# jxhe/vae-lagging-encoder

Measured on AMD Instinct MI355X. Metric: aggressive-loop seqs/sec, higher is better.
Workload: dtype bf16

## Files before the change

include/lvae.h:

```cpp
#ifndef LVAE_H
#define LVAE_H

#include <stdint.h>

#ifdef __cplusplus
extern "C" {
#endif

int lv_gemm_f32(int transA, int transB, int M, int N, int K, float alpha,
                const float* A, long lda, const float* B, long ldb, float* C, long ldc, int accumulate,
                const float* add1, long ld1, int mod1, const float* add2, long ld2, int mod2,
                float* ws , long ws_floats, void* stream);

int lv_gemm_bf16(int transA, int transB, int M, int N, int K, float alpha,
                 const float* A, long lda, const float* B, long ldb, float* C, long ldc, int accumulate,
                 const float* add1, long ld1, int mod1, const float* add2, long ld2, int mod2,
                 float* ws, long ws_floats, void* stream);

int lv_gemm_b16(int transA, int M, int N, int K, float alpha,
                const uint16_t* A, long lda, const uint16_t* B, long ldb, float* C, long ldc, int accumulate,
                const float* add1, long ld1, int mod1, const float* add2, long ld2, int mod2,
                float* ws, long ws_floats, void* stream);
int lv_gemm_b16_dual_supported(int M, int N, int K, long ws_floats);
int lv_gemm_b16_dual(int transA, int M, int N, int K, const uint16_t* A, long lda, const uint16_t* B, long ldb,
// ... 208 lines not shown

int lv_tanh_f32(const float* in, float* out, long n, void* stream);
int lv_colsum_f32(const float* in, long ld, int R, int C, float* out, float* out2, void* stream);
int lv_add_f32(const float* a, const float* b, float* out, long n, void* stream);
int lv_sum_accum_f32(const float* x, long n, float* out_dev, void* stream);
int lv_add_scalar_f32(float* x_dev, float v, void* stream);

int lv_sumsq_workspace_floats(void);
int lv_sumsq_f32(const float* x, long n, float* ws, float* out_dev, int accumulate, void* stream);
int lv_clip_coef_f32(const float* sumsq_dev, float max_norm, float* coef_dev, float* norm_out_dev, void* stream);
int lv_clip_norm2_f32(const float* g1, long n1, const float* g2, long n2, float* ws, float max_norm,
                      float* sumsq_dev, float* coef_dev, float* norm_dev, void* stream);
int lv_sgd_step_f32(float* p, float* g, long n, const float* lr_dev, const float* coef_dev, int write_back_clipped,
                    void* stream);
int lv_scale_f32(float* x, long n, const float* coef_dev, void* stream);
int lv_clip_norm2_txn_f32(const float* g1, long n1, const float* g2, long n2, float* ws, float max_norm,
                          float* sumsq_dev, float* coef_dev, float* norm_dev, const int* status1, const int* status2,
                          const float* guard, float* txn, float* acc, void* stream);
int lv_clip_norm2_fold_txn_f32(const float* g1, long n1, const float* g2, long n2, float* ws, const float* extra, int n_extra,
                               float max_norm, float* sumsq_dev, float* coef_dev, float* norm_dev, const int* status1,
                               const int* status2, const float* guard, float* txn, float* acc, void* stream);
int lv_clip_coef_txn_f32(const float* sumsq_dev, float max_norm, float* coef_dev, float* norm_out_dev, const int* status1,
                         const int* status2, const float* guard, float* txn, float* acc, void* stream);
int lv_txn_guard_f32(const int* status1, const int* status2, float* guard, void* stream);
int lv_sgd_step_txn_f32(float* p, float* g, long n, const float* lr_dev, const float* coef_dev, int write_back_clipped,
                        const float* void_flag_dev, void* stream);
int lv_scale_txn_f32(float* x, long n, const float* coef_dev, const float* void_flag_dev, void* stream);
int lv_sgd_step_scale_txn_f32(float* p, float* g, long n, const float* lr_dev, const float* coef_dev, int write_back_clipped,
                              float* x2, long n2, const float* void_flag_dev, void* stream);
int lv_sgd_step_scale_rows_txn_f32(float* p, float* g, long n, const float* lr_dev, const float* coef_dev, int write_back_clipped,
                                   float* x2, long n2, const float* void_flag_dev, long emb_off, int V, int ni, const int* sorted_tok,
                                   int N, void* stream);
int lv_sgd_momentum_step_f32(float* p, float* g, float* buf, long n, const float* lr_dev, const float* coef_dev, float momentum,
                             int write_back_clipped, void* stream);
int lv_sgd_momentum_step_txn_f32(float* p, float* g, float* buf, long n, const float* lr_dev, const float* coef_dev, float momentum,
                                 int write_back_clipped, const float* void_flag_dev, void* stream);
int lv_sgd_momentum_step_scale_txn_f32(float* p, float* g, float* buf, long n, const float* lr_dev, const float* coef_dev, float momentum,
                                       int write_back_clipped, float* x2, long n2, const float* void_flag_dev, void* stream);
int lv_adam_step_f32(float* p, float* g, float* m, float* v, long n, const float* lr_dev, const float* coef_dev,
                     const float* step_dev, float beta1, float beta2, float eps, int write_back_clipped, void* stream);
int lv_adam_step_txn_f32(float* p, float* g, float* m, float* v, long n, const float* lr_dev, const float* coef_dev, float* step_dev,
                         double beta1, double beta2, float eps, int write_back_clipped, const float* void_flag_dev, void* stream);
int lv_adam_step_scale_txn_f32(float* p, float* g, float* m, float* v, long n, const float* lr_dev, const float* coef_dev,
                               float* step_dev, double beta1, double beta2, float eps, int write_back_clipped, float* x2, long n2,
                               const float* void_flag_dev, void* stream);

int lv_rng_normal_f32(float* out, long n, const uint64_t* state_dev, uint64_t substream, void* stream);
int lv_rng_keepmask_u8(uint8_t* out, long n, float keep_prob, const uint64_t* state_dev, uint64_t substream, void* stream);
int lv_rng_advance(uint64_t* state_dev, uint64_t inc, void* stream);
int lv_rng_noise_step(float* eps, long n_eps, uint8_t* mask_in, long n_in, float keep_in, uint8_t* mask_out, long n_out,
                      float keep_out, uint64_t* state_dev, uint64_t inc, void* stream);
int lv_rng_bernoulli_f32(const float* p, float* out, long n, const uint64_t* state_dev, uint64_t substream,
                         void* stream);

int lv_gauss_logpdf_f32(const float* z, const float* mu, const float* logvar, float* out, int B, int ns, int nz, void* stream);
int lv_logsumexp_rows_f32(const float* in, long ld, int R, int C, float add, float* out, void* stream);
int lv_calc_mi_f32(const float* mu, const float* logvar, const float* z, float* ws, float* out_dev, int Bx, int Bz, int nz,
                   void* stream);
int lv_au_accum_f32(const float* mu, const float* mean, float* acc_dev, int B, int nz, void* stream);

int lv_dec_cond_ll_f32_supported(int V, int ni, int H, int nz, int T);
long lv_dec_cond_ll_f32_ws_floats(int V, int H, int nz, int B, int T);
int lv_dec_cond_ll_f32(const int64_t* x, int B, int T, const float* z, long z_stride, int K, const float* embed,
                       const float* trans, const float* w_ih, const float* w_hh, const float* b_ih, const float* b_hh,
                       const float* pred, int V, int ni, int H, int nz, float* ws, float* cond_ll, void* stream);
int lv_grid_posterior_f32(const float* cond_ll, const float* z, long z_stride, int B, int K, int nz, float* log_post,
                          float* mean, void* stream);

int lv_mh_chain_f32_supported(int V, int ni, int H, int nz, int T);
long lv_mh_chain_f32_ws_floats(int V, int H, int nz, int B, int T);
int lv_mh_chain_prep_f32(const int64_t* x, int B, int T, const float* embed, const float* trans, const float* w_ih,
                         const float* w_hh, const float* b_ih, const float* b_hh, const float* pred, int V, int ni, int H, int nz,
                         float* ws, void* stream);
int lv_mh_chain_f32(const int64_t* x, int B, int T, const float* ws, int V, int H, int nz, int C, float* cur, float* cur_ll,
                    int* accepts, const float* eps, const float* u, int n_iter, int iter0, int burn_in, int thin, int nsamples,
                    float std, int first, float* samples, float* ratio_out, int* accept_out, void* stream);
int lv_mh_step_f32(const float* cond_ll, float* prop, float* cur, float* cur_ll, int* accepts, const float* u,
                   const float* eps_next, float std, float* samples, int rows, int C, int nz, int nsamples, int keep, int init,
                   float* ratio_out, int* accept_out, void* stream);

int lv_ais_chain_f32_supported(int V, int ni, int H, int nz, int T);
int lv_ais_chain_f32(const int64_t* x, int B, int T, const float* ws, int V, int H, int nz, int C, float* cur, float* g_cur,
                     float* lq_cur, double* logw, int* accepts, const float* eps, const float* u, const double* beta,
                     const float* std_it, const float* mu0, const float* lv0, int n_iter, int first, float* ratio_out,
                     int* accept_out, double* logw_out, void* stream);
int lv_ais_step_f32(const float* cond_ll, float* prop, float* cur, float* g_cur, float* lq_cur, double* logw, int* accepts,
                    const float* u, double beta, const float* eps_next, float std_next, double dbeta_next, const float* mu0,
                    const float* lv0, int rows, int C, int nz, int init, float* ratio_out, int* accept_out,
                    double* logw_out_next, void* stream);

int lv_hmc_leap_f32(const float* rec, const float* dz, int parts, float* pos, float* mom, float* k0, float* cur, float* g_cur,
                    float* lq_cur, float* rec_cur, float* d_cur, double* logw, int* accepts, float* eps, const float* u,
                    const float* mom_next, double beta, double beta_next, double dbeta_next, const float* mu0, const float* lv0,
                    int rows, int C, int nz, int L, int mode, float up, float down, float eps_min, float eps_max, float* dh_out,
                    int* flag_out, double* logw_out_next, float* keep_out, void* stream);

int lv_argmax_rows_f32(const float* in, long ld, int R, int C, int64_t* idx, void* stream);
int lv_log_softmax_rows_f32(const float* in, long ld, int R, int C, const float* addrow, float* out, long ldo, void* stream);
int lv_sample_rows_f32(const float* in, long ld, int R, int C, const float* u, int64_t* idx, void* stream);
int lv_sample_filtered_rows_f32(const float* in, long ld, int R, int C, const float* u, float inv_temp, int top_k, float top_p,
                                int64_t* idx, float* lp, float* lq, int* kept, float* tau, int* ntie, void* stream);

int lv_im2col_f32(const float* x, float* col, long ldcol, int N, int H, int W, int C, int Ho, int Wo,
                  int kh, int kw, int pad, int stride, int ntaps, void* stream);
int lv_col2im_f32(const float* dcol, long ldcol, float* dx, int N, int H, int W, int C, int Ho, int Wo,
                  int kh, int kw, int pad, int stride, int ntaps, int accumulate, void* stream);
// ... 104 lines not shown
```

vae_lagging_encoder_amd/_lib.py:

```python
import ctypes
import os
import threading

from . import build as _build

_vp = ctypes.c_void_p
_i = ctypes.c_int
_l = ctypes.c_long
_f = ctypes.c_float
_d = ctypes.c_double
_u64 = ctypes.c_uint64

SIGNATURES = {
    "lv_gemm_f32": [_i, _i, _i, _i, _i, _f, _vp, _l, _vp, _l, _vp, _l, _i, _vp, _l, _i, _vp, _l, _i, _vp, _l, _vp],
    "lv_gemm_bf16": [_i, _i, _i, _i, _i, _f, _vp, _l, _vp, _l, _vp, _l, _i, _vp, _l, _i, _vp, _l, _i, _vp, _l, _vp],
    "lv_gemm_b16": [_i, _i, _i, _i, _f, _vp, _l, _vp, _l, _vp, _l, _i, _vp, _l, _i, _vp, _l, _i, _vp, _l, _vp],
    "lv_gemm_h16": [_i, _i, _i, _f, _vp, _l, _vp, _l, _vp, _l, _i, _vp, _l, _i, _vp, _l, _i, _vp, _l, _vp],
    "lv_gemm_b16_dual_supported": [_i, _i, _i, _l],
    "lv_gemm_b16_dual": [_i, _i, _i, _i, _vp, _l, _vp, _l, _vp, _l, _i, _vp, _l, _vp, _l, _vp],
    "lv_gemm_b16_pair_supported": [_i, _i, _i, _i, _i, _i, _i, _i, _l],
    "lv_gemm_b16_pair_pending": [_vp, _vp],
    "lv_gemm_b16_pair": [_i, _i, _i, _i, _vp, _l, _vp, _l, _vp, _l, _i, _vp, _l,
                         _i, _i, _i, _i, _vp, _l, _vp, _l, _vp, _l, _vp, _l, _vp],
    "lv_gemm_b16_keep": [_i, _i, _i, _vp, _l, _vp, _l, _vp, _vp, _f, _i, _vp, _l, _vp],
    "lv_gemm_b16_sumsq_parts": [_i, _i, _i, _l],
    "lv_gemm_b16_sumsq": [_i, _i, _i, _i, _vp, _l, _vp, _l, _vp, _l, _vp, _l, _vp, _i, _vp],
    "lv_gemm_b16_nll_parts": [_i],
    "lv_gemm_b16_tile": [_i, _i, _i, _i, _i, _f, _vp, _l, _vp, _l, _vp, _l, _i, _vp, _l, _i, _vp, _l, _i, _vp, _l, _vp],
    "lv_gemm_b16_nll_tile": [_i, _i, _i, _i, _vp, _l, _vp, _l, _vp, _l, _vp, _l, _i, _i, _vp, _vp, _vp],
    "lv_gemm_b16_nll": [_i, _i, _i, _vp, _l, _vp, _l, _vp, _l, _vp, _l, _i, _i, _vp, _vp, _vp],
    "lv_softmax_nll_merge_f32": [_vp, _i, _vp, _vp, _vp, _i, _vp],
    "lv_softmax_nll_bwd_h16": [_vp, _l, _vp, _vp, _l, _i, _vp, _vp, _l, _i, _i, _i, _vp],
    "lv_cvt_bf16_f32": [_vp, _l, _i, _i, _vp, _l, _vp, _l, _vp],
    "lv_cvt_bf16_keep_f32": [_vp, _l, _i, _i, _i, _vp, _f, _vp, _l, _vp, _l, _vp],
    "lv_cvt_bf16_hs3_f32": [_vp, _l, _i, _i, _i, _vp, _f, _vp, _l, _vp, _l, _vp, _l, _vp],
    "lv_cvt_f32_bf16_scaled": [_vp, _l, _f, _vp, _vp],
    "lv_keep_scale_f32": [_vp, _vp, _f, _i, _i, _i, _vp],
    "lv_cvt_bf16_gates_f32": [_vp, _l, _i, _i, _vp, _l, _vp, _l, _vp],
    "lv_cvt_bf16_lo_f32": [_vp, _l, _i, _i, _i, _vp, _l, _i, _i, _vp, _l, _vp, _l, _vp],
    "lv_cvt_h16_f32": [_vp, _l, _i, _i, _i, _vp, _l, _i, _i, _vp, _l, _vp, _l, _vp],
    "lv_gate_interleave_f32": [_vp, _vp, _i, _i, _vp, _vp],
    "lv_lstm_fwd_bf16_ug": [_vp, _vp, _vp, _vp, _vp, _vp, _f, _vp, _vp, _i, _i, _i, _vp],
    "lv_lstm_fwd_f32_ug": [_vp, _vp, _vp, _vp, _vp, _vp, _f, _vp, _vp, _i, _i, _i, _vp],
    "lv_loss_assemble_f32": [_vp, _vp, _vp, _vp, _vp, _vp, _vp, _vp, _vp, _i, _i, _vp],
    "lv_loss_assemble_rng_f32": [_vp, _vp, _vp, _vp, _vp, _vp, _vp, _vp, _vp, _i, _i, _vp, _u64, _vp],
    "lv_gx_expand_add_f32": [_vp, _vp, _vp, _i, _i, _i, _i, _vp],
    "lv_sample_sum_f32": [_vp, _vp, _i, _i, _i, _i, _vp],
    "lv_sample_sum_b16": [_vp, _l, _vp, _l, _i, _i, _i, _i, _vp],
    "lv_repeat_rows_i64": [_vp, _vp, _i, _i, _i, _vp],
    "lv_loss_assemble_ns_f32": [_vp, _vp, _vp, _vp, _vp, _vp, _vp, _vp, _vp, _i, _i, _i, _vp],
    "lv_loss_assemble_ns_rng_f32": [_vp, _vp, _vp, _vp, _vp, _vp, _vp, _vp, _vp, _i, _i, _i, _vp, _u64, _vp],
    "lv_loss_assemble_iw_f32": [_vp] * 13 + [_i, _i, _i, _i, _vp],
    "lv_loss_assemble_iw_rng_f32": [_vp] * 13 + [_i, _i, _i, _i, _vp, _u64, _vp],
    "lv_reparam_iw_bwd_f32": [_vp, _vp, _vp, _vp, _i, _i, _i, _vp],
    "lv_enc_head_iw_bwd_f32": [_vp, _vp, _vp, _i, _vp, _vp, _vp, _vp, _vp, _vp, _i, _i, _i, _i, _vp],
    "lv_loss_assemble_dreg_f32": [_vp] * 14 + [_i, _i, _i, _i, _vp],
    "lv_loss_assemble_dreg_rng_f32": [_vp] * 14 + [_i, _i, _i, _i, _vp, _u64, _vp],
    "lv_reparam_iwdz_bwd_f32": [_vp, _vp, _vp, _vp, _vp, _vp, _i, _i, _i, _vp],
    "lv_enc_head_dreg_bwd_f32": [_vp, _vp, _vp, _i, _vp, _vp, _vp, _vp, _vp, _vp, _vp, _i, _i, _i, _i, _vp],
    "lv_kl_freebits_fwd_f32": [_vp, _f, _i, _vp, _vp, _vp, _i, _i, _vp],
    "lv_reparam_kl_gated_bwd_f32": [_vp, _vp, _vp, _vp, _vp, _vp, _i, _i, _i, _vp],
    "lv_loss_assemble_fb_f32": [_vp] * 10 + [_i, _i, _i, _vp],
    "lv_loss_assemble_fb_rng_f32": [_vp] * 10 + [_i, _i, _i, _vp, _u64, _vp],
    "lv_enc_head_gated_bwd_f32": [_vp, _vp, _vp, _i, _vp, _vp, _vp, _vp, _vp, _vp, _vp, _i, _i, _i, _i, _vp],
    "lv_enc_head_fwd_f32": [_vp, _vp, _vp, _vp, _vp, _vp, _i, _i, _i, _i, _vp],
    "lv_enc_head_bwd_f32": [_vp, _vp, _vp, _i, _vp, _vp, _vp, _vp, _vp, _vp, _i, _i, _i, _i, _vp],
    "lv_dec_tail_parts": [_i],
    "lv_dec_init_f32": [_vp, _vp, _vp, _l, _i, _vp, _vp, _vp, _vp, _vp, _i, _i, _i, _i, _vp],
    "lv_dec_tail_bwd_f32": [_vp, _vp, _vp, _vp, _l, _i, _vp, _vp, _l, _vp, _vp, _vp, _vp, _i, _i, _i, _vp],
    "lv_dec_tail_dz_f32": [_vp, _vp, _vp, _l, _i, _vp, _vp, _i, _i, _i, _vp],
    "lv_svi_step_f32": [_vp, _vp, _i, _vp, _vp, _vp, _f, _f, _f, _vp, _vp, _vp, _vp, _vp, _vp, _vp, _i, _i, _i, _vp],
    "lv_svi_rec_step_f32": [_vp, _i, _vp, _vp, _f, _f, _f, _vp, _vp, _vp, _vp, _vp, _vp, _i, _i, _i, _vp],
    "lv_savae_adjoint_f32": [_vp, _vp, _vp, _vp, _vp, _f, _f, _f, _f, _vp, _vp, _vp, _vp, _i, _i, _i, _vp],
    "lv_savae_hvp_f32": [_vp, _i, _vp, _vp, _vp, _vp, _vp, _vp, _i, _i, _i, _vp],
    "lv_clip_norm2_f32": [_vp, _l, _vp, _l, _vp, _f, _vp, _vp, _vp, _vp],
    "lv_clip_norm2_txn_f32": [_vp, _l, _vp, _l, _vp, _f, _vp, _vp, _vp, _vp, _vp, _vp, _vp, _vp, _vp],
    "lv_clip_norm2_fold_txn_f32": [_vp, _l, _vp, _l, _vp, _vp, _i, _f, _vp, _vp, _vp, _vp, _vp, _vp, _vp, _vp, _vp],
    "lv_clip_coef_txn_f32": [_vp, _f, _vp, _vp, _vp, _vp, _vp, _vp, _vp, _vp],
    "lv_txn_guard_f32": [_vp, _vp, _vp, _vp],
    "lv_sgd_step_txn_f32": [_vp, _vp, _l, _vp, _vp, _i, _vp, _vp],
    "lv_scale_txn_f32": [_vp, _l, _vp, _vp, _vp],
    "lv_sgd_step_scale_txn_f32": [_vp, _vp, _l, _vp, _vp, _i, _vp, _l, _vp, _vp],
    "lv_sgd_step_scale_rows_txn_f32": [_vp, _vp, _l, _vp, _vp, _i, _vp, _l, _vp, _l, _i, _i, _vp, _i, _vp],
    "lv_sgd_momentum_step_f32": [_vp, _vp, _vp, _l, _vp, _vp, _f, _i, _vp],
    "lv_sgd_momentum_step_txn_f32": [_vp, _vp, _vp, _l, _vp, _vp, _f, _i, _vp, _vp],
    "lv_sgd_momentum_step_scale_txn_f32": [_vp, _vp, _vp, _l, _vp, _vp, _f, _i, _vp, _l, _vp, _vp],
    "lv_rng_noise_step": [_vp, _l, _vp, _l, _f, _vp, _l, _f, _vp, _u64, _vp],
    "lv_lstm_persist16_wpk_floats": [],
    "lv_lstm_persist16_xch_floats": [],
    "lv_lstm_persist16_xch_clear": [_vp, _vp],
    "lv_lstm_persist16_saved_floats": [_i, _i],
    "lv_lstm_persist16_pack": [_vp, _vp, _i, _i, _vp],
    "lv_lstm_persist16_import_saved": [_vp, _vp, _vp, _i, _i, _i, _i, _vp],
    "lv_lstm_persist16_pack2": [_vp, _vp, _vp, _i, _vp],
# ... 213 lines not shown
```

vae_lagging_encoder_amd/csrc/lv_gemm_b16.hip:

```cpp
#if defined(LV_TRACE)
#define lv_trace_buf lv_trace_buf_gemm
#endif
#include "lv_device.h"
#if defined(LV_TRACE) && !defined(LV_EMU)
__device__ unsigned long long* lv_trace_buf = nullptr;
extern "C" int lv_trace_set_gemm(void* p) { return (int)hipMemcpyToSymbol(HIP_SYMBOL(lv_trace_buf), &p, sizeof(p)); }
#endif
#include <type_traits>

namespace {

#ifndef LV_B16_ABL
#define LV_B16_ABL 0
#endif
#ifndef LV_B16_SPLIT_TARGET
#define LV_B16_SPLIT_TARGET 512
#endif

constexpr int BK = 64;
constexpr int BT = 128;
constexpr int NCH = BK / 8;

#ifndef LV_NLL_ABL
#define LV_NLL_ABL 0
#endif
struct GemmQ {
    const uint16_t* A; const uint16_t* B; float* C;
    int M, N, K;
    long lda, ldb, ldc;
    float alpha;
    int accumulate;
    const float* add1; long ld1; int mod1;
    const float* add2; long ld2; int mod2;
    int tilesM, tilesN;
    int splits, kt_per_split;
    float* ws;
    uint16_t* C16; long ldc16;
    const int64_t* ids; long ids_stride; int tgt_off; int Bsz;
    float2* part; int nparts;
    float* tgt;
    const uint8_t* keep; float kscale; int keepT;
    float* sq; int sq_only;
    float* C2; long ldc2; int nsplit;
};

__device__ __forceinline__ uint4 load_chunk(const uint16_t* __restrict__ p, int valid) {
    if (valid >= 8) return *reinterpret_cast<const uint4*>(p);
    uint32_t h[8];
#pragma unroll
    for (int e = 0; e < 8; ++e) h[e] = e < valid ? (uint32_t)p[e] : 0u;
    uint4 q;
    q.x = h[0] | (h[1] << 16); q.y = h[2] | (h[3] << 16); q.z = h[4] | (h[5] << 16); q.w = h[6] | (h[7] << 16);
    return q;
}


// ... 1505 lines not shown
            }
            sr[u] = grs[u] < R ? grs[u] : R - 1;
        }
        if (gids) {
#pragma unroll
            for (int u = 0; u < 8; ++u) sr[u] = gids[(long)bbs[u] * gstride + (grs[u] < R ? tts[u] : 0)];
#pragma unroll
            for (int u = 0; u < 8; ++u) sr[u] = sr[u] < 0 ? 0 : (sr[u] >= gV ? gV - 1 : sr[u]);
        }
        float v[8];
        uint8_t kp[8];
#pragma unroll
        for (int u = 0; u < 8; ++u) v[u] = src[sr[u] * lds_ + gcc];
        if (keep) {
#pragma unroll
            for (int u = 0; u < 8; ++u) kp[u] = keep[((long)bbs[u] * Tt + (grs[u] < R ? tts[u] : 0)) * C + gcc];
        }
#pragma unroll
        for (int u = 0; u < 8; ++u) {
            const int gr = grs[u];
            uint16_t b = 0;
            if (gr < R && gc < C) {
                float x = v[u];
                if (keep) {
                    if (gids) x = kp[u] ? x * kscale : 0.f;
                    else x *= kp[u] ? kscale : 0.f;
                }
                b = (uint16_t)lv_f32_to_bf16_bits(x);
                if (lo == 1) b = (uint16_t)lv_f32_to_bf16_bits(x - lv_bf16_bits_to_f32(b));
                if (dst) {
                    const long dr = gate_H > 0 ? (long)(gr % gate_H) * 4 + gr / gate_H : gr;
                    dst[dr * ldd + gc] = lo == 2 ? lv_f32_to_f16_bits(lv_sat_f16(x)) : b;
                }
            }
            tile[q + 4 * (i0 + u)][lane] = b;
        }
    }
    if (!dstT) return;
    __syncthreads();
#pragma unroll 4
    for (int i = 0; i < 16; ++i) {
        const int c = q + 4 * i;
        const int gc = c0 + c, gr = r0 + lane;
        if (gc < C && gr < R) dstT[(long)gc * ldt + gr] = tile[lane][c];
    }
}


__global__ __launch_bounds__(256) void cvt_b16_v4_kernel(const float* __restrict__ src, long lds_, int R, int C,
                                                         uint16_t* __restrict__ dst, long ldd, uint16_t* __restrict__ dstT, long ldt,
                                                         int gate_H, const uint8_t* __restrict__ keep, float kscale, int Bsz,
                                                         const int64_t* __restrict__ gids, long gstride, int gV, int lo) {
    __shared__ __attribute__((aligned(8))) uint16_t tile[64][68];
    const int t = (int)threadIdx.x;
    const int r0 = (int)blockIdx.y * 64, c0 = (int)blockIdx.x * 64;
    const int q = t >> 4, cl = t & 15;
    const bool tb = keep || gids;
    const int Tt = tb ? R / Bsz : 1;
    int bb = tb ? (r0 + q) % Bsz : 0, tt = tb ? (r0 + q) / Bsz : 0;
    const int gc = c0 + 4 * cl;
    const int gcc = gc < C ? gc : C - 4;
    int grs[4], bbs[4], tts[4];
    long sr[4];
#pragma unroll
    for (int u = 0; u < 4; ++u) {
        grs[u] = r0 + q + 16 * u;
        bbs[u] = bb; tts[u] = tt;
        if (tb) {
            bb += 16;
            while (bb >= Bsz) { bb -= Bsz; ++tt; }
        }
        sr[u] = grs[u] < R ? grs[u] : R - 1;
    }
    if (gids) {
#pragma unroll
        for (int u = 0; u < 4; ++u) sr[u] = gids[(long)bbs[u] * gstride + (grs[u] < R ? tts[u] : 0)];
#pragma unroll
        for (int u = 0; u < 4; ++u) sr[u] = sr[u] < 0 ? 0 : (sr[u] >= gV ? gV - 1 : sr[u]);
    }
    float4 v[4];
    uint32_t kp[4] = {0u, 0u, 0u, 0u};
#pragma unroll
    for (int u = 0; u < 4; ++u) v[u] = *reinterpret_cast<const float4*>(src + sr[u] * lds_ + gcc);
    if (keep) {
#pragma unroll
        for (int u = 0; u < 4; ++u)
            kp[u] = *reinterpret_cast<const uint32_t*>(keep + ((long)bbs[u] * Tt + (grs[u] < R ? tts[u] : 0)) * C + gcc);
    }
#pragma unroll
    for (int u = 0; u < 4; ++u) {
        const int gr = grs[u];
        uint16_t b[4] = {0, 0, 0, 0}, d[4] = {0, 0, 0, 0};
        const bool in = gr < R && gc < C;
        if (in) {
            const float xs[4] = {v[u].x, v[u].y, v[u].z, v[u].w};
#pragma unroll
            for (int e = 0; e < 4; ++e) {
                float x = xs[e];
                if (keep) {
                    const bool k = (kp[u] >> (8 * e)) & 0xFFu;
                    if (gids) x = k ? x * kscale : 0.f;
                    else x *= k ? kscale : 0.f;
                }
                b[e] = (uint16_t)lv_f32_to_bf16_bits(x);
                if (lo == 1) b[e] = (uint16_t)lv_f32_to_bf16_bits(x - lv_bf16_bits_to_f32(b[e]));
                d[e] = lo == 2 ? lv_f32_to_f16_bits(lv_sat_f16(x)) : b[e];
            }
            if (dst) {
                const long dr = gate_H > 0 ? (long)(gr % gate_H) * 4 + gr / gate_H : gr;
                *reinterpret_cast<uint2*>(dst + dr * ldd + gc) = make_uint2((uint32_t)d[0] | ((uint32_t)d[1] << 16), (uint32_t)d[2] | ((uint32_t)d[3] << 16));
            }
        }
        *reinterpret_cast<uint2*>(&tile[q + 16 * u][4 * cl]) = make_uint2((uint32_t)b[0] | ((uint32_t)b[1] << 16), (uint32_t)b[2] | ((uint32_t)b[3] << 16));
    }
    if (!dstT) return;
    __syncthreads();
    const int rl = t & 15, gr = r0 + 4 * rl;
#pragma unroll
    for (int i = 0; i < 4; ++i) {
        const int c = q + 16 * i, gct = c0 + c;
        const uint16_t e0 = tile[4 * rl][c], e1 = tile[4 * rl + 1][c], e2 = tile[4 * rl + 2][c], e3 = tile[4 * rl + 3][c];
        if (gct < C) {
            uint16_t* o = dstT + (long)gct * ldt + gr;
            if (gr + 3 < R) *reinterpret_cast<uint2*>(o) = make_uint2((uint32_t)e0 | ((uint32_t)e1 << 16), (uint32_t)e2 | ((uint32_t)e3 << 16));
            else {
                if (gr < R) o[0] = e0;
                if (gr + 1 < R) o[1] = e1;
                if (gr + 2 < R) o[2] = e2;
            }
        }
    }
}

__global__ __launch_bounds__(256) void cvt_b16_hs3_kernel(const float* __restrict__ src, long lds_, int T, int Bsz, int C,
                                                          const uint8_t* __restrict__ keep, float kscale,
                                                          uint16_t* __restrict__ dst, long ldd, uint16_t* __restrict__ dstT, long ldt,
                                                          uint16_t* __restrict__ hT, long ldh) {
    __shared__ __attribute__((aligned(8))) uint16_t tile[2][64][68];
    const int t = (int)threadIdx.x;
    const int r0 = (int)blockIdx.y * 64, c0 = (int)blockIdx.x * 64;
    const int q = t >> 4, cl = t & 15;
    const int RO = T * Bsz, R = RO + Bsz;
    const int ko = keep ? 1 : 0;
    int bb = (r0 + q) % Bsz, tt = (r0 + q) / Bsz;
    const int gc = c0 + 4 * cl;
    const int gcc = gc < C ? gc : C - 4;
    int grs[4], bbs[4], tts[4];
#pragma unroll
    for (int u = 0; u < 4; ++u) {
        grs[u] = r0 + q + 16 * u;
        bbs[u] = bb; tts[u] = tt;
        bb += 16;
        while (bb >= Bsz) { bb -= Bsz; ++tt; }
    }
    float4 v[4];
    uint32_t kp[4] = {0u, 0u, 0u, 0u};
#pragma unroll
    for (int u = 0; u < 4; ++u) v[u] = *reinterpret_cast<const float4*>(src + (long)(grs[u] < R ? grs[u] : R - 1) * lds_ + gcc);
    if (keep) {
#pragma unroll
        for (int u = 0; u < 4; ++u) {
            const bool out_row = grs[u] < R && tts[u] >= 1;
            kp[u] = *reinterpret_cast<const uint32_t*>(keep + ((long)(out_row ? bbs[u] : 0) * T + (out_row ? tts[u] - 1 : 0)) * C + gcc);
        }
    }
#pragma unroll
    for (int u = 0; u < 4; ++u) {
        const int gr = grs[u];
        uint16_t b[4] = {0, 0, 0, 0}, d[4] = {0, 0, 0, 0};
        if (gr < R && gc < C) {
            const float xs[4] = {v[u].x, v[u].y, v[u].z, v[u].w};
#pragma unroll
            for (int e = 0; e < 4; ++e) {
                float x = xs[e];
                b[e] = (uint16_t)lv_f32_to_bf16_bits(x);
                if (keep) {
                    x *= ((kp[u] >> (8 * e)) & 0xFFu) ? kscale : 0.f;
                    d[e] = (uint16_t)lv_f32_to_bf16_bits(x);
                } else d[e] = b[e];
            }
            if (gr >= Bsz)
                *reinterpret_cast<uint2*>(dst + (long)(gr - Bsz) * ldd + gc) = make_uint2((uint32_t)d[0] | ((uint32_t)d[1] << 16), (uint32_t)d[2] | ((uint32_t)d[3] << 16));
        }
        *reinterpret_cast<uint2*>(&tile[0][q + 16 * u][4 * cl]) = make_uint2((uint32_t)b[0] | ((uint32_t)b[1] << 16), (uint32_t)b[2] | ((uint32_t)b[3] << 16));
        if (keep)
            *reinterpret_cast<uint2*>(&tile[1][q + 16 * u][4 * cl]) = make_uint2((uint32_t)d[0] | ((uint32_t)d[1] << 16), (uint32_t)d[2] | ((uint32_t)d[3] << 16));
    }
    __syncthreads();
    const int rl = t & 15, gr = r0 + 4 * rl;
    const bool otv = (Bsz & 3) == 0;
#pragma unroll
    for (int i = 0; i < 4; ++i) {
        const int c = q + 16 * i, gct = c0 + c;
        if (gct >= C) continue;
        {
            const uint16_t e0 = tile[0][4 * rl][c], e1 = tile[0][4 * rl + 1][c], e2 = tile[0][4 * rl + 2][c], e3 = tile[0][4 * rl + 3][c];
            uint16_t* o = hT + (long)gct * ldh + gr;
            if (gr + 3 < RO) *reinterpret_cast<uint2*>(o) = make_uint2((uint32_t)e0 | ((uint32_t)e1 << 16), (uint32_t)e2 | ((uint32_t)e3 << 16));
            else {
                if (gr < RO) o[0] = e0;
                if (gr + 1 < RO) o[1] = e1;
                if (gr + 2 < RO) o[2] = e2;
            }
        }
        {
            const uint16_t e0 = tile[ko][4 * rl][c], e1 = tile[ko][4 * rl + 1][c], e2 = tile[ko][4 * rl + 2][c], e3 = tile[ko][4 * rl + 3][c];
            uint16_t* orow = dstT + (long)gct * ldt;
            if (otv && gr >= Bsz && gr + 3 < R)
                *reinterpret_cast<uint2*>(orow + (gr - Bsz)) = make_uint2((uint32_t)e0 | ((uint32_t)e1 << 16), (uint32_t)e2 | ((uint32_t)e3 << 16));
            else {
                if (gr >= Bsz && gr < R) orow[gr - Bsz] = e0;
                if (gr + 1 >= Bsz && gr + 1 < R) orow[gr + 1 - Bsz] = e1;
                if (gr + 2 >= Bsz && gr + 2 < R) orow[gr + 2 - Bsz] = e2;
                if (gr + 3 >= Bsz && gr + 3 < R) orow[gr + 3 - Bsz] = e3;
            }
        }
    }
}

static void cvt_launch(void* stream, const float* src, long lds, int R, int C, uint16_t* dst, long ldd, uint16_t* dstT, long ldt, int gate_H,
                       const uint8_t* keep, float kscale, int Bsz, const int64_t* gids, long gstride, int gV, int lo) {
    const dim3 grid((unsigned)lv_cdiv(C, 64), (unsigned)lv_cdiv(R, 64)), block(256);
    const bool v4 = C >= 4 && C % 4 == 0 && lds % 4 == 0 && (((uintptr_t)src) & 15) == 0 &&
                    (!dst || (ldd % 4 == 0 && (((uintptr_t)dst) & 7) == 0)) && (!dstT || (ldt % 4 == 0 && (((uintptr_t)dstT) & 7) == 0)) &&
                    (!keep || (((uintptr_t)keep) & 3) == 0);
    if (v4) LV_LAUNCH(cvt_b16_v4_kernel, grid, block, 0, stream, src, lds, R, C, dst, ldd, dstT, ldt, gate_H, keep, kscale, Bsz, gids, gstride, gV, lo);
    else LV_LAUNCH(cvt_b16_kernel, grid, block, 0, stream, src, lds, R, C, dst, ldd, dstT, ldt, gate_H, keep, kscale, Bsz, gids, gstride, gV, lo);
}

}

static bool t256_wanted(int tile, int M, int N, int K) {
    if (tile) return tile >= 256;
    return 2.0 * M * N * K >= 1.0e11 && M >= 1024 && N >= 1024 && K >= 1024;
}
#ifndef LV_B16_SCHED_DEFAULT
#define LV_B16_SCHED_DEFAULT -1
#endif
static int t256_sched(int tile, int kt_per_wg) {
    if (tile >= 256) return tile - 256;
    return LV_B16_SCHED_DEFAULT >= 0 ? LV_B16_SCHED_DEFAULT : (kt_per_wg >= 24 ? 2 : 1);
}

static Tail256 t256_plan(long tiles, int nk, long ws_floats) {
    Tail256 q;
    q.full = (int)(tiles / 256 * 256);
    q.tail_s = 1;
    q.kt_per_piece = nk;
    const long tail = tiles - q.full;
    q.tail = (int)tail;
    if (tail == 0) return q;
    double best = (double)nk * 2.0;
    for (int s = 2; s <= 16; ++s) {
        if (nk / s < 4 || tail * s * (long)(BT2 * BT2) > ws_floats) break;
        const double cost = (double)lv_cdiv(tail * s, 256) * lv_cdiv(nk, s) * 2.0 + (s + 1) * tail * 0.058;
        if (cost < best) { best = cost; q.tail_s = s; }
    }
    q.kt_per_piece = lv_cdiv(nk, q.tail_s);
    q.tail_s = lv_cdiv(nk, q.kt_per_piece);
    return q;
}

extern "C" int lv_keep_scale_f32(float* x, const uint8_t* keep, float kscale, int T, int Bsz, int C, void* stream);

static int gemm_b16_launch(int tile, int transA, int M, int N, int K, float alpha,
                           const uint16_t* A, long lda, const uint16_t* B, long ldb,
                           float* C, long ldc, int accumulate,
                           const float* add1, long ld1, int mod1,
                           const float* add2, long ld2, int mod2,
                           float* ws, long ws_floats, void* stream, const uint8_t* keep, float kscale, int Bsz,
                           float* sq = nullptr, int sq_only = 0, int f16 = 0, float* C2 = nullptr, long ldc2 = 0, int nsplit = 0) {
    if (tile != 0 && tile != 128 && (tile < 256 || tile > 258)) return LV_ERR_ARG;
    if (f16) {
        if (transA || keep || sq || !LV_B16_GLDS) return LV_ERR_UNSUPPORTED;
        tile = 128;
    }
    if (M < 0 || N < 0 || K < 0) return LV_ERR_SHAPE;
    if (M == 0 || N == 0) return LV_OK;
// ... 371 lines not shown
```

vae_lagging_encoder_amd/csrc/lv_head.hip:

```cpp
#include "lv_device.h"

namespace {

template <class FA, class FB> __device__ __forceinline__ float dot2_batched(int n, FA a, FB b) {
    float s0 = 0.f, s1 = 0.f;
    int i = 0;
    for (; i + 7 < n; i += 8) {
        float x[8], y[8];
#pragma unroll
        for (int u = 0; u < 8; ++u) { x[u] = a(i + u); y[u] = b(i + u); }
#pragma unroll
        for (int u = 0; u < 8; u += 2) { s0 = fmaf(x[u], y[u], s0); s1 = fmaf(x[u + 1], y[u + 1], s1); }
    }
    for (; i + 1 < n; i += 2) { s0 = fmaf(a(i), b(i), s0); s1 = fmaf(a(i + 1), b(i + 1), s1); }
    if (i < n) s0 = fmaf(a(i), b(i), s0);
    return s0 + s1;
}

template <class Src, class Put> __device__ __forceinline__ void stage_batched(int n, int tid, Src src, Put put) {
    for (int i0 = tid; i0 < n; i0 += 256 * 8) {
        float v[8];
#pragma unroll
        for (int u = 0; u < 8; ++u) { const int i = i0 + 256 * u; v[u] = *src(i < n ? i : n - 1); }
#pragma unroll
        for (int u = 0; u < 8; ++u) { const int i = i0 + 256 * u; if (i < n) put(i, v[u]); }
    }
}

__global__ __launch_bounds__(256) void enc_head_fwd_kernel(const float* __restrict__ hT, const float* __restrict__ wlin,
                                                           const float* __restrict__ eps, float* __restrict__ mulv,
                                                           float* __restrict__ z, float* __restrict__ kl,
                                                           int H, int ns, int nz) {
    LV_DYN_SHARED(smem);
    float* sh = reinterpret_cast<float*>(smem);
    float* sm = sh + H;
    float* sk = sm + 2 * nz;
    const int b = (int)blockIdx.x, tid = (int)threadIdx.x, l = tid & 63, w = tid >> 6;
    const int nz2 = 2 * nz;
    for (int h = tid; h < H; h += 256) sh[h] = hT[(long)b * H + h];
    __syncthreads();
    for (int o0 = 0; o0 < nz2; o0 += 64) {
        float acc[16];
#pragma unroll
        for (int i = 0; i < 16; ++i) acc[i] = 0.f;
#pragma unroll 4
        for (int h = l; h < H; h += 64) {
            const float x = sh[h];
#pragma unroll
            for (int i = 0; i < 16; ++i) {
                const int o = o0 + w + 4 * i;
                acc[i] = fmaf(x, wlin[(long)(o < nz2 ? o : 0) * H + h], acc[i]);
            }
        }
#pragma unroll
        for (int i = 0; i < 16; ++i) {
            const int o = o0 + w + 4 * i;
            const float s = lv_wave_sum(acc[i]);
            if (l == 0 && o < nz2) { sm[o] = s; mulv[(long)b * nz2 + o] = s; }
        }
    }
    __syncthreads();
    for (int j = tid; j < nz; j += 256) {
        const float m = sm[j], lv = sm[nz + j];
        const float sd = expf(0.5f * lv);
        sk[j] = (m * m + expf(lv)) - lv - 1.f;
        for (int s = 0; s < ns; ++s) {
            const long zi = ((long)b * ns + s) * nz + j;
            z[zi] = m + eps[zi] * sd;
        }
    }
    __syncthreads();
    if (tid == 0) {
        float s = 0.f;
        for (int j = 0; j < nz; ++j) s += sk[j];
        kl[b] = 0.5f * s;
    }
}

__device__ __forceinline__ const float* head_gate(const float* g) { return g; }

enum { HEAD_PLAIN = 0, HEAD_IW = 1, HEAD_DREG = 2 };
template <int HB_COLS, int MODE, class... Gate>
__global__ __launch_bounds__(256) void enc_head_bwd_kernel(const float* __restrict__ mulv, const float* __restrict__ eps,
                                                           const float* __restrict__ dz, int parts, const float* __restrict__ dkl,
                                                           const float* __restrict__ hT, const float* __restrict__ wlin,
                                                           float* __restrict__ dmulv, float* __restrict__ dhT,
                                                           float* __restrict__ gwlin, int B, int H, int ns, int nz, Gate... gate) {
    LV_DYN_SHARED(smem);
    const int nz2 = 2 * nz;
    float* sd = reinterpret_cast<float*>(smem);
    float* sw = sd + B * nz2;
    float* shh = sw + nz2 * HB_COLS;
    const int tid = (int)threadIdx.x;
    const int h0 = (int)blockIdx.x * HB_COLS;
    const long pstride = (long)B * ns * nz;
    stage_batched(nz2 * HB_COLS, tid,
                  [&](int i) { const int j = i / HB_COLS, c = i % HB_COLS; return wlin + (long)j * H + (h0 + c < H ? h0 + c : H - 1); },
                  [&](int i, float v) { sw[i] = h0 + i % HB_COLS < H ? v : 0.f; });
    stage_batched(B * HB_COLS, tid,
                  [&](int i) { const int bb = i / HB_COLS, c = i % HB_COLS; return hT + (long)bb * H + (h0 + c < H ? h0 + c : H - 1); },
                  [&](int i, float v) { shh[i] = h0 + i % HB_COLS < H ? v : 0.f; });
    float* sg = shh + B * HB_COLS;
    const int ne = B * ns * nz;
    const bool v4 = (ne & 3) == 0 && (pstride & 3) == 0 && (((uintptr_t)dz) & 15) == 0;
    if (v4) {
        for (int e = 4 * tid; e < ne; e += 1024) {
            float4 g = make_float4(0.f, 0.f, 0.f, 0.f);
            for (int q0 = 0; q0 < parts; q0 += 16) {
                float4 pv[16];
#pragma unroll
                for (int u = 0; u < 16; ++u) pv[u] = *reinterpret_cast<const float4*>(dz + (long)(q0 + u < parts ? q0 + u : 0) * pstride + e);
#pragma unroll
                for (int u = 0; u < 16; ++u)
                    if (q0 + u < parts) { g.x += pv[u].x; g.y += pv[u].y; g.z += pv[u].z; g.w += pv[u].w; }
            }
            sg[e] = g.x; sg[e + 1] = g.y; sg[e + 2] = g.z; sg[e + 3] = g.w;
        }
    } else
    for (int e = tid; e < ne; e += 512) {
        const int e1 = e + 256 < ne ? e + 256 : e;
        float g0 = 0.f, g1 = 0.f;
        for (int q0 = 0; q0 < parts; q0 += 32) {
            float pa[32], pb[32];
#pragma unroll
            for (int u = 0; u < 32; ++u) {
                const long off = (long)(q0 + u < parts ? q0 + u : 0) * pstride;
                pa[u] = dz[off + e];
                pb[u] = dz[off + e1];
            }
// ... 276 lines not shown
```

vae_lagging_encoder_amd/csrc/lv_lstm.hip:

```cpp
#include "lv_device.h"

namespace {

static inline int h_round_up(int x, int m) { return (x + m - 1) / m * m; }

template <int MB> struct RecNit { static constexpr int value = MB <= 2 ? 16 : (MB == 4 ? 8 : 4); };

template <int MB, int NIT>
__device__ __forceinline__ void rec_mm_core(const float* __restrict__ ap, long a_qpitch,
                                            const float* __restrict__ wp, int it0, int it1, int l, f32x4 (&acc)[MB]) {
    const int i = l & 15, kq = l >> 4;
    const float* a_lane = ap + i * 4;
    const float* w_lane = wp + i * 4;
    for (int itb = it0; itb < it1; itb += NIT) {
        float4 wv[NIT];
        float4 av[NIT][MB];
        if (itb + NIT <= it1) {
#pragma unroll
            for (int u = 0; u < NIT; ++u) {
                const long q = 4 * (itb + u) + kq;
                wv[u] = *reinterpret_cast<const float4*>(w_lane + q * 64);
#pragma unroll
                for (int mb = 0; mb < MB; ++mb) av[u][mb] = *reinterpret_cast<const float4*>(a_lane + q * a_qpitch + mb * 64);
                LV_SCHED_BARRIER();
            }
        } else {
#pragma unroll
            for (int u = 0; u < NIT; ++u) {
                const bool ok = itb + u < it1;
                const long q = ok ? 4 * (itb + u) + kq : 4 * it0 + kq;
                const float4 t = *reinterpret_cast<const float4*>(w_lane + q * 64);
                wv[u] = ok ? t : make_float4(0.f, 0.f, 0.f, 0.f);
#pragma unroll
                for (int mb = 0; mb < MB; ++mb) av[u][mb] = *reinterpret_cast<const float4*>(a_lane + q * a_qpitch + mb * 64);
            }
        }
        LV_SCHED_BARRIER();
#pragma unroll
        for (int u = 0; u < NIT; ++u) {
#pragma unroll
            for (int mb = 0; mb < MB; ++mb) acc[mb] = lv_mfma_16x16x4(av[u][mb].x, wv[u].x, acc[mb]);
#pragma unroll
            for (int mb = 0; mb < MB; ++mb) acc[mb] = lv_mfma_16x16x4(av[u][mb].y, wv[u].y, acc[mb]);
#pragma unroll
            for (int mb = 0; mb < MB; ++mb) acc[mb] = lv_mfma_16x16x4(av[u][mb].z, wv[u].z, acc[mb]);
#pragma unroll
            for (int mb = 0; mb < MB; ++mb) acc[mb] = lv_mfma_16x16x4(av[u][mb].w, wv[u].w, acc[mb]);
        }
    }
}

template <int MB, int NIT>
__device__ __forceinline__ void rec_mm_core_bf16(const uint4* __restrict__ ap, long a_opitch,
// ... 588 lines not shown
                                    int tanh_init, int T, int B, int H, void* stream) {
    return lstm_bwd_impl<true>(dh_ext, dh_last, dmask, dscale, whh, gates, hs, cs, dG, dGsum, ws, dh0, dc0, tanh_init,
                               T, B, H, stream, dG16);
}

extern "C" int lv_lstm_fwd_bf16_ug(const float* gx, const float* whh, float* hs, float* cs, float* gates,
                                   const uint8_t* dmask, float dscale, float* hdrop, float* ws,
                                   int T, int B, int H, void* stream) {
    return lstm_fwd_impl<true>(gx, whh, hs, cs, gates, dmask, dscale, hdrop, ws, T, B, H, stream, 1);
}

extern "C" int lv_lstm_fwd_f32_ug(const float* gx, const float* whh, float* hs, float* cs, float* gates,
                                  const uint8_t* dmask, float dscale, float* hdrop, float* ws,
                                  int T, int B, int H, void* stream) {
    return lstm_fwd_impl<false>(gx, whh, hs, cs, gates, dmask, dscale, hdrop, ws, T, B, H, stream, 1);
}

extern "C" int lv_lstm_fwd_len_f32(const float* gx, const float* whh, float* hs, float* cs, float* gates,
                                   const uint8_t* dmask, float dscale, float* hdrop, float* ws,
                                   const int* steps, int max_steps, int T, int B, int H, void* stream) {
    return lstm_fwd_impl<false, true>(gx, whh, hs, cs, gates, dmask, dscale, hdrop, ws, T, B, H, stream, 0, steps, max_steps);
}

extern "C" int lv_lstm_bwd_len_f32(const float* dh_ext, const float* dh_last, const uint8_t* dmask, float dscale,
                                   const float* whh, const float* gates, const float* hs, const float* cs,
                                   float* dG, float* dGsum, float* ws, float* dh0, float* dc0, int tanh_init,
                                   const int* steps, int max_steps, int T, int B, int H, void* stream) {
    return lstm_bwd_impl<false, true>(dh_ext, dh_last, dmask, dscale, whh, gates, hs, cs, dG, dGsum, ws, dh0, dc0, tanh_init,
                                      T, B, H, stream, nullptr, steps, max_steps);
}

namespace {
__global__ __launch_bounds__(256) void nll_mask_len_kernel(float* __restrict__ nll, const int* __restrict__ steps, long n, int B) {
    const long idx = (long)blockIdx.x * 256 + threadIdx.x;
    if (idx >= n) return;
    const int t = (int)(idx / B), b = (int)(idx % B);
    if (t >= steps[b]) nll[idx] = 0.f;
}
}

extern "C" int lv_nll_mask_len_f32(float* nll, const int* steps, int max_steps, int T, int B, void* stream) {
    if (!nll || !steps) return LV_ERR_ARG;
    if (T < 0 || B <= 0 || max_steps < 0 || max_steps > T) return LV_ERR_SHAPE;
    if (T == 0) return LV_OK;
    const long n = (long)T * B;
    LV_LAUNCH(nll_mask_len_kernel, dim3((unsigned)lv_cdiv(n, 256)), dim3(256), 0, stream, nll, steps, n, B);
    LV_CHECK_LAUNCH();
    return LV_OK;
}

namespace {
__global__ __launch_bounds__(256) void gate_interleave_kernel(const float* __restrict__ a, const float* __restrict__ b,
                                                              long n, int H, float* __restrict__ out) {
    const long idx = (long)blockIdx.x * 256 + threadIdx.x;
    if (idx >= n) return;
    const long r = idx / (4L * H);
    const int c = (int)(idx % (4L * H));
    const long src = r * 4L * H + (long)(c & 3) * H + (c >> 2);
    out[idx] = a[src] + (b ? b[src] : 0.f);
}
}

extern "C" int lv_gate_interleave_f32(const float* a, const float* b, int R, int H, float* out, void* stream) {
    if (!a || !out || R < 0 || H <= 0) return LV_ERR_ARG;
    if (R == 0) return LV_OK;
    const long n = (long)R * 4 * H;
    LV_LAUNCH(gate_interleave_kernel, dim3((unsigned)lv_cdiv(n, 256)), dim3(256), 0, stream, a, b, n, H, out);
    LV_CHECK_LAUNCH();
    return LV_OK;
}
```

vae_lagging_encoder_amd/csrc/lv_lstm_persist16.hip:

```cpp
#include "lv_device.h"
#include "lv_persist_common.h"

#if defined(LV_TRACE) && !defined(LV_EMU)
__device__ unsigned long long* lv_trace_buf = nullptr;
extern "C" int lv_trace_set(void* p) { return (int)hipMemcpyToSymbol(HIP_SYMBOL(lv_trace_buf), &p, sizeof(p)); }
#endif

#ifndef LV_RS_Q
#define LV_RS_Q 2
#endif
#ifndef LV_P16_ABL
#define LV_P16_ABL 0
#endif

namespace {

using namespace lvp;

__device__ __forceinline__ float abl_u2f(uint32_t u) { float f; memcpy(&f, &u, 4); return f; }

constexpr int HP16 = PH / 2 + 8;
constexpr int DP16 = 64 + 8;
constexpr int RED_SLOTS = 33;
constexpr int SAVED_PER_ROW = 160;
constexpr int RS16_SLOTS_MAX = 256;
template <int V> struct lv_const { static constexpr int value = V; };

__global__ __launch_bounds__(256) void pack_w_k16_kernel(const float* __restrict__ whh, uint4* __restrict__ wpk, int f16);
__global__ __launch_bounds__(256) void pack_w_rs16_kernel(const float* __restrict__ whh, uint4* __restrict__ wpk);

__device__ __forceinline__ void pack_w_k16_one(const float* __restrict__ whh, uint4* __restrict__ wpk, long idx, int f16 = 0) {
    const int l = (int)(idx & 63), nb = (int)((idx >> 6) & 7), ks = (int)((idx >> 9) & 7);
    const int wave_id = (int)(idx >> 12), m = wave_id >> 2, w = wave_id & 3;
    const int c = l & 15, kq = l >> 4, col = 16 * nb + c;
    const float* row = whh + ((long)(col & 3) * PH + 32 * m + (col >> 2)) * PH + 256 * w + 32 * ks + 8 * kq;
    if (f16) {
        float r[8];
#pragma unroll
        for (int e = 0; e < 8; ++e) r[e] = lv_sat_f16(row[e]);
        wpk[idx] = make_uint4(lv_pack_f16x2(r[0], r[1]), lv_pack_f16x2(r[2], r[3]), lv_pack_f16x2(r[4], r[5]), lv_pack_f16x2(r[6], r[7]));
    }
    else
        wpk[idx] = make_uint4(lv_pack_bf16x2(row[0], row[1]), lv_pack_bf16x2(row[2], row[3]), lv_pack_bf16x2(row[4], row[5]),
                              lv_pack_bf16x2(row[6], row[7]));
}
__device__ __forceinline__ void pack_w_rs16_one(const float* __restrict__ whh, uint4* __restrict__ wpk, long idx) {
    const int l = (int)(idx & 63), nb = (int)((idx >> 6) & 15), ks = (int)((idx >> 10) & 3);
    const int wave_id = (int)(idx >> 12), m = wave_id >> 2, w = wave_id & 3;
    const int c = l & 15, kq = l >> 4, j = 256 * w + 16 * nb + c;
    float v[8];
#pragma unroll
    for (int e = 0; e < 8; ++e) {
        const int n2 = 32 * ks + 8 * kq + e;
        v[e] = whh[((long)(n2 & 3) * PH + 32 * m + (n2 >> 2)) * PH + j];
    }
    wpk[idx] = make_uint4(lv_pack_bf16x2(v[0], v[1]), lv_pack_bf16x2(v[2], v[3]), lv_pack_bf16x2(v[4], v[5]), lv_pack_bf16x2(v[6], v[7]));
}
__global__ __launch_bounds__(256) void pack_w_both16_kernel(const float* __restrict__ whh, uint4* __restrict__ wfwd, uint4* __restrict__ wbwd,
                                                            int fwd_f16) {
    const long n = 128L * 64 * 64;
    const long idx = (long)blockIdx.x * 256 + threadIdx.x;
    if (idx < n) pack_w_k16_one(whh, wfwd, idx, fwd_f16);
    else if (idx < 2 * n) pack_w_rs16_one(whh, wbwd, idx - n);
}

__global__ __launch_bounds__(256) void pack_w_k16_kernel(const float* __restrict__ whh, uint4* __restrict__ wpk, int f16) {
    const long idx = (long)blockIdx.x * 256 + threadIdx.x;
    if (idx < 128L * 8 * 8 * 64) pack_w_k16_one(whh, wpk, idx, f16);
}
__global__ __launch_bounds__(256) void pack_w_rs16_kernel(const float* __restrict__ whh, uint4* __restrict__ wpk) {
    const long idx = (long)blockIdx.x * 256 + threadIdx.x;
    if (idx < 128L * 4 * 16 * 64) pack_w_rs16_one(whh, wpk, idx);
}

struct Fwd16P {
    const float* gx; const uint4* wpk;
    float* hs; float* cs; float* saved;
    gran_t* hx;
    int* status;
    int T, B, R;
    uint4* clr; long clr_n;
    const uint16_t* x16; long ldx; const uint16_t* wih; const float* add; long add_ld;
};

__device__ __forceinline__ void clear_other_half(uint4* q, long n) {
    if (!q) return;
    const long stride = (long)gridDim.x * blockDim.x;
    for (long i = (long)blockIdx.x * blockDim.x + threadIdx.x; i < n; i += stride) q[i] = make_uint4(0u, 0u, 0u, 0u);
}

template <int RP> struct Cfg16 {
    static constexpr int NP = RP > 8 ? 2 : 1;
    static constexpr int SBK = RP > 8 ? 4 : 8;
    static constexpr int SBB = 8;
};

template <int RP>
struct __attribute__((aligned(16))) Fwd16Lds {
    uint32_t hl[RP * HP16];
    f32x4 red[2][4][RP][RED_SLOTS];
    uint32_t dump[256];
    int abort;
};

constexpr int XNI = 512;
constexpr int XKS = XNI / 32;
constexpr int XKL = 12;
constexpr int XS_PITCH = XNI / 8 + 2;
struct __attribute__((aligned(16))) Fwd16XLds : Fwd16Lds<4> {
    uint4 wih[4][XKL][2][64];
    uint4 xs[16 * XS_PITCH];
    f32x4 rb[2][16][RED_SLOTS];
};
template <bool C, class A, class B> struct lv_pick_t { typedef A type; };
template <class A, class B> struct lv_pick_t<false, A, B> { typedef B type; };

// ... 839 lines not shown
```

vae_lagging_encoder_amd/csrc/lv_rng.hip:

```cpp
#include "lv_device.h"

namespace {

struct U4 { uint32_t x, y, z, w; };

__device__ __forceinline__ void mulhilo(uint32_t a, uint32_t b, uint32_t& hi, uint32_t& lo) {
    const uint64_t p = (uint64_t)a * (uint64_t)b;
    hi = (uint32_t)(p >> 32);
    lo = (uint32_t)p;
}

__device__ __forceinline__ U4 philox4x32_10(U4 c, uint32_t k0, uint32_t k1) {
#pragma unroll
    for (int r = 0; r < 10; ++r) {
        uint32_t hi0, lo0, hi1, lo1;
        mulhilo(0xD2511F53u, c.x, hi0, lo0);
        mulhilo(0xCD9E8D57u, c.z, hi1, lo1);
        U4 n;
        n.x = hi1 ^ c.y ^ k0;
        n.y = lo1;
        n.z = hi0 ^ c.w ^ k1;
        n.w = lo0;
        c = n;
        k0 += 0x9E3779B9u;
        k1 += 0xBB67AE85u;
    }
    return c;
}

__device__ __forceinline__ U4 draw(const uint64_t* state, uint64_t substream, uint64_t i) {
    const uint64_t seed = state[0], off = state[1];
    U4 c;
    c.x = (uint32_t)i;
    c.y = (uint32_t)(i >> 32);
    c.z = (uint32_t)off ^ (uint32_t)(substream << 20);
    c.w = (uint32_t)(off >> 32) ^ (uint32_t)(substream >> 12);
    return philox4x32_10(c, (uint32_t)seed, (uint32_t)(seed >> 32));
}

__device__ __forceinline__ float u01(uint32_t x) { return ((float)(x >> 8) + 0.5f) * (1.0f / 16777216.0f); }

__global__ __launch_bounds__(256) void rng_normal_kernel(float* __restrict__ out, long n, const uint64_t* __restrict__ state,
                                                         uint64_t substream) {
    const long i = (long)blockIdx.x * 256 + threadIdx.x;
    if (i * 4 >= n) return;
    const U4 r = draw(state, substream, (uint64_t)i);
    const float u1 = u01(r.x), u2 = u01(r.y), u3 = u01(r.z), u4 = u01(r.w);
    const float r1 = sqrtf(-2.f * logf(u1)), r2 = sqrtf(-2.f * logf(u3));
    const float t1 = 6.283185307179586f * u2, t2 = 6.283185307179586f * u4;
    const float v[4] = {r1 * cosf(t1), r1 * sinf(t1), r2 * cosf(t2), r2 * sinf(t2)};
    for (int j = 0; j < 4; ++j)
        if (i * 4 + j < n) out[i * 4 + j] = v[j];
}

__global__ __launch_bounds__(256) void rng_keepmask_kernel(uint8_t* __restrict__ out, long n, float keep,
                                                           const uint64_t* __restrict__ state, uint64_t substream) {
    const long i = (long)blockIdx.x * 256 + threadIdx.x;
    if (i * 8 >= n) return;
    const U4 r = draw(state, substream, (uint64_t)i);
    const uint32_t thr = (uint32_t)(keep * 65536.0f);
    const uint32_t w[4] = {r.x, r.y, r.z, r.w};
    for (int j = 0; j < 8; ++j) {
        const uint32_t h = (w[j >> 1] >> ((j & 1) * 16)) & 0xFFFFu;
        if (i * 8 + j < n) out[i * 8 + j] = (h < thr) ? 1 : 0;
    }
}

__global__ __launch_bounds__(256) void rng_bernoulli_kernel(const float* __restrict__ p, float* __restrict__ out, long n,
                                                            const uint64_t* __restrict__ state, uint64_t substream) {
    const long i = (long)blockIdx.x * 256 + threadIdx.x;
    if (i * 4 >= n) return;
    const U4 r = draw(state, substream, (uint64_t)i);
    const float u[4] = {u01(r.x), u01(r.y), u01(r.z), u01(r.w)};
    for (int j = 0; j < 4; ++j)
        if (i * 4 + j < n) out[i * 4 + j] = (u[j] < p[i * 4 + j]) ? 1.f : 0.f;
}

__global__ void rng_advance_kernel(uint64_t* state, uint64_t inc) {
    if (threadIdx.x == 0 && blockIdx.x == 0) state[1] += inc;
}

struct NoiseP {
    float* eps; long n_eps;
    uint8_t* m1; long n1; float keep1;
    uint8_t* m2; long n2; float keep2;
    uint64_t* state; uint64_t inc;
    unsigned nb0, nb1;
};

__global__ __launch_bounds__(256) void rng_noise_step_kernel(NoiseP p) {
    const unsigned bid = blockIdx.x;
    const int tid = (int)threadIdx.x;
    if (bid < p.nb0) {
        const long i = (long)bid * 256 + tid;
        if (i * 4 < p.n_eps) {
            const U4 r = draw(p.state, 0, (uint64_t)i);
            const float u1 = u01(r.x), u2 = u01(r.y), u3 = u01(r.z), u4 = u01(r.w);
            const float r1 = sqrtf(-2.f * logf(u1)), r2 = sqrtf(-2.f * logf(u3));
            const float t1 = 6.283185307179586f * u2, t2 = 6.283185307179586f * u4;
            const float v[4] = {r1 * cosf(t1), r1 * sinf(t1), r2 * cosf(t2), r2 * sinf(t2)};
            for (int j = 0; j < 4; ++j)
                if (i * 4 + j < p.n_eps) p.eps[i * 4 + j] = v[j];
        }
    } else {
        const bool first = bid < p.nb0 + p.nb1;
        uint8_t* out = first ? p.m1 : p.m2;
        const long n = first ? p.n1 : p.n2;
        const long i = (long)(bid - p.nb0 - (first ? 0u : p.nb1)) * 256 + tid;
        if (i * 8 < n) {
            const U4 r = draw(p.state, first ? 1 : 2, (uint64_t)i);
            const uint32_t thr = (uint32_t)((first ? p.keep1 : p.keep2) * 65536.0f);
            const uint32_t w[4] = {r.x, r.y, r.z, r.w};
            if (i * 8 + 8 <= n && ((((uintptr_t)out) & 7) == 0)) {
                uint32_t lo = 0, hi = 0;
                for (int j = 0; j < 4; ++j) {
                    lo |= (((w[j >> 1] >> ((j & 1) * 16)) & 0xFFFFu) < thr ? 1u : 0u) << (8 * j);
                    hi |= (((w[2 + (j >> 1)] >> ((j & 1) * 16)) & 0xFFFFu) < thr ? 1u : 0u) << (8 * j);
                }
                *reinterpret_cast<uint2*>(out + i * 8) = make_uint2(lo, hi);
            } else {
                for (int j = 0; j < 8; ++j) {
                    const uint32_t h = (w[j >> 1] >> ((j & 1) * 16)) & 0xFFFFu;
                    if (i * 8 + j < n) out[i * 8 + j] = (h < thr) ? 1 : 0;
                }
            }
        }
    }
}

}

extern "C" int lv_rng_normal_f32(float* out, long n, const uint64_t* state, uint64_t substream, void* stream) {
    if (!out || !state || n < 0) return LV_ERR_ARG;
    if (n == 0) return LV_OK;
    LV_LAUNCH(rng_normal_kernel, dim3((unsigned)lv_cdiv((n + 3) / 4, 256)), dim3(256), 0, stream, out, n, state, substream);
    LV_CHECK_LAUNCH();
    return LV_OK;
}

extern "C" int lv_rng_keepmask_u8(uint8_t* out, long n, float keep_prob, const uint64_t* state, uint64_t substream,
                                  void* stream) {
    if (!out || !state || n < 0) return LV_ERR_ARG;
    if (n == 0) return LV_OK;
    LV_LAUNCH(rng_keepmask_kernel, dim3((unsigned)lv_cdiv((n + 7) / 8, 256)), dim3(256), 0, stream, out, n, keep_prob, state,
              substream);
    LV_CHECK_LAUNCH();
    return LV_OK;
}

extern "C" int lv_rng_bernoulli_f32(const float* p, float* out, long n, const uint64_t* state, uint64_t substream,
                                    void* stream) {
    if (!p || !out || !state || n < 0) return LV_ERR_ARG;
    if (n == 0) return LV_OK;
    LV_LAUNCH(rng_bernoulli_kernel, dim3((unsigned)lv_cdiv((n + 3) / 4, 256)), dim3(256), 0, stream, p, out, n, state, substream);
    LV_CHECK_LAUNCH();
    return LV_OK;
}

extern "C" int lv_rng_advance(uint64_t* state, uint64_t inc, void* stream) {
    if (!state) return LV_ERR_ARG;
    LV_LAUNCH(rng_advance_kernel, dim3(1), dim3(64), 0, stream, state, inc);
    LV_CHECK_LAUNCH();
    return LV_OK;
}

extern "C" int lv_rng_noise_step(float* eps, long n_eps, uint8_t* mask_in, long n_in, float keep_in, uint8_t* mask_out,
                                 long n_out, float keep_out, uint64_t* state, uint64_t inc, void* stream) {
    if (!eps || !state || n_eps < 0 || n_in < 0 || n_out < 0) return LV_ERR_ARG;
    if (!mask_in) n_in = 0;
    if (!mask_out) n_out = 0;
    NoiseP p{eps, n_eps, mask_in, n_in, keep_in, mask_out, n_out, keep_out, state, inc,
             (unsigned)lv_cdiv((n_eps + 3) / 4, 256), (unsigned)lv_cdiv((n_in + 7) / 8, 256)};
    const unsigned nb = p.nb0 + p.nb1 + (unsigned)lv_cdiv((n_out + 7) / 8, 256);
    if (nb > 0) LV_LAUNCH(rng_noise_step_kernel, dim3(nb), dim3(256), 0, stream, p);
    if (inc != 0) LV_LAUNCH(rng_advance_kernel, dim3(1), dim3(64), 0, stream, state, inc);
    LV_CHECK_LAUNCH();
    return LV_OK;
}
```

vae_lagging_encoder_amd/engine.py:

```python
import ctypes
import math
import numbers
import os

import numpy as np
import torch

from . import _lib

def backend_for(device):
    device = torch.device(device)
    if device.type == "cuda":
        return _lib.load()
    raise _lib.LvaeError(
        "vae_lagging_encoder_amd runs on MI355X (ROCm 'cuda' tensors) through its HIP extension; got a %s tensor. "
        "There is no CPU fallback." % device.type)


def stream_ptr(device):
    device = torch.device(device)
    if device.type == "cuda":
        return ctypes.c_void_p(torch.cuda.current_stream(device).cuda_stream)
    return None

# ... 331 lines not shown

def status_ptr(eng):
    return P(eng.status) if eng.status is not None else None


_PERSIST_H = 1024
_PERSIST_MAX_B = 128


def _persist_rows(eng, B):
    rows = getattr(eng, "persist_rows", None)
    if rows is not None and 8 * rows >= B and 1 <= rows <= 16:
        return int(rows)
    return (B + 7) // 8


def _saved_floats(eng, T, B, H):
    n = T * B * 4 * H
    if H == _PERSIST_H and eng.precision == "bf16" and eng.persistent and B <= _PERSIST_MAX_B:
        n = max(n, eng.lib.lv_lstm_persist16_saved_floats(T, _persist_rows(eng, B)))
    return n


def _persistent_ok(eng, img, B, H, device, max_b):
    return (eng.precision == "bf16" and img is not None and eng.persistent and H == _PERSIST_H and B <= max_b
            and torch.device(device).type == "cuda" and torch.cuda.get_device_properties(device).multi_processor_count >= 256)


FUSED_GX = os.environ.get("LVAE_FUSED_GX", "1") != "0"
FUSED_GX_ENC = True
FUSED_GX_DEC = True
_FUSED_GX_NI = 512


def _fused_gx_ok(eng, img, B, H, ni, device, layer_on):
    if not (FUSED_GX and layer_on and ni == _FUSED_GX_NI and eng.ws_evictable and _persistent_ok(eng, img, B, H, device, _PERSIST_MAX_B)):
        return False
    if _persist_rows(eng, B) > 4:
        return False
    return not (torch.cuda.is_current_stream_capturing() or (eng._wimg is not None and getattr(eng._wimg, "xstate", {}).get("captured")))


def _gx_buffer(c, w, rows, H):
    if w.Gx is None:
        w.Gx = c.f32(rows, 4 * H)
        c.grew(w.ws_key, rows * 4 * H * 4)
    return w.Gx


def weights_version(eng):
    return (sum(p._version for p in eng.flat.params), eng.wgen)


def _weight_images(eng, lib, s, device, want_persist, lstm=True, pred=False):
    wi = eng._wimg
    V, ni, H = eng.dims()[:3]
    v = eng.flat.views
    c = eng.wsc
    if wi is None:
        wi = eng._wimg = _NS()
        wi.ver = object()
        wi.W = wi.WT = wi.pred = wi.predT = wi.fwd16 = wi.bwd16 = wi.xch = None
        if lstm:
            wi.W = c.i16(4 * H, ni)
            wi.WT = c.i16(ni, 4 * H)
        wi.ldv = _round_up(V, 32)
        if pred:
            wi.pred = c.i16(V, H)
            wi.predT = c.i16(H, wi.ldv)
        wi.packed16 = False
    ver = weights_version(eng) if eng.cache_weight_images else object()
    h16 = bool(getattr(eng, "_h16_now", False))
    stale = wi.ver != ver or getattr(wi, "h16", False) != h16
    if stale:
        wih = v["lstm.weight_ih_l0"]
        if wi.W is not None and h16:
            lib.lv_cvt_h16_f32(P(wih), wih.shape[1], 4 * H, ni, H, None, 0, 1, 0, P(wi.W), ni, P(wi.WT), 4 * H, s)
        elif wi.W is not None:
            lib.lv_cvt_bf16_gates_f32(P(wih), wih.shape[1], H, ni, P(wi.W), ni, P(wi.WT), 4 * H, s)
        wi.h16 = h16
        if wi.pred is not None:
            lib.lv_cvt_bf16_f32(P(v["pred_linear.weight"]), H, V, H, P(wi.pred), H, P(wi.predT), wi.ldv, s)
        wi.ver = ver
        wi.packed16 = False
    if want_persist and not wi.packed16:
        if wi.fwd16 is None:
            n = lib.lv_lstm_persist16_wpk_floats()
            wi.fwd16, wi.bwd16 = c.f32(n), c.f32(n)
            wi.xch = torch.zeros(lib.lv_lstm_persist16_xch_floats(), dtype=torch.float32, device=c.device)
            wi.xstate = {"f": 0, "g": 0, "gcls": [0, 0]}
        (lib.lv_lstm_persist16_pack2_h16 if h16 else lib.lv_lstm_persist16_pack2)(P(v["lstm.weight_hh_l0"]), P(wi.fwd16), P(wi.bwd16), H, s)
        wi.packed16 = True
    return wi


def _xch_flags(wi, kind, rows, device, T=1):
    st = wi.xstate
    if T <= 0:
        return 0
    if torch.device(device).type == "cuda" and torch.cuda.is_current_stream_capturing():
        st["captured"] = True
    if st.get("captured"):
        return 0
    half = st[kind]
    st[kind] = 1 - half
    fl = 2 | (half << 2)
    if kind == "g":
        cls = 1 if rows <= 4 else (2 if rows <= 8 else 3)
        fl |= st["gcls"][1 - half] << 3
        st["gcls"][half] = cls
        st["gcls"][1 - half] = 0
    return fl


class SeqLengths(object):

    def __init__(self, lengths, B, T, device):
        if torch.is_tensor(lengths):
            if lengths.dtype not in (torch.int64, torch.int32, torch.int16, torch.int8, torch.uint8) or lengths.dim() != 1:
                raise ValueError("sentence lengths: a 1-D integer tensor or a list of ints expected, got %s %s"
                                 % (lengths.dtype, tuple(lengths.shape)))
            host = [int(v) for v in lengths.detach().cpu().tolist()]
        else:
            try:
                host = list(lengths)
            except TypeError:
                raise ValueError("sentence lengths: a 1-D integer tensor or a list of ints expected, got %r" % (type(lengths),))
            if not all(isinstance(v, int) and not isinstance(v, bool) for v in host):
                raise ValueError("sentence lengths: a list of ints expected")
        if len(host) != B:
            raise ValueError("sentence lengths: %d values for a batch of %d sentences" % (len(host), B))
        if B > 0 and min(host) < 2:
            raise ValueError("sentence lengths: every sentence holds at least <s> and </s>; got a length of %d" % min(host))
        if B > 0 and max(host) > T:
            raise ValueError("sentence lengths: a length of %d in a batch tensor of %d columns" % (max(host), T))
        self.host, self.B, self.T = host, B, T
        self.device = torch.device(device)
        self.max = max(host) if host else 0
        self.enc = torch.tensor(host, dtype=torch.int32).to(self.device)
        self._dec = {}

    def dec(self, ns=1):
        d = self._dec.get(ns)
        if d is None:
# ... 130 lines not shown
_PERSIST_BWD_MAX_B = 128


def check_persistent_status(eng):
    st = eng.status
    if st is not None and int(st.item()) != 0:
        raise _lib.LvaeError("persistent LSTM kernel reported hand-off timeout (status %d) on ladder rung %d (%s): not all 256 "
                             "workgroups were resident (e.g. another kernel held compute units for seconds), or -- with "
                             "eng.persist_flags bit 0 set -- a group's workgroups were not placed on one XCD.  The fused trainers "
                             "recover from this by themselves (engine.demote_persistent); on the drop-in autograd path call it and "
                             "redo the step" % (int(st.item()), persist_rung(eng), PERSIST_RUNGS[persist_rung(eng)]))


def _need_canonical_saved(w):
    lay = getattr(w, "saved_layout", None)
    if lay is not None and lay[0] != "canonical":
        raise _lib.LvaeError("the saved activations are in the 16-row persistent kernels' own order %r, but the backward was routed to a "
                             "kernel that reads gates [T][B][4H] / cs: eng.persistent / eng.persist_rows changed between forward and "
                             "backward" % (lay,))


def _lstm_backward(eng, lib, s, img, w, dh_ext, dh_last, mask, scale, whh, dh0, dc0, tanh_init, T, B, H, device, steps=None):
    if steps is not None:
        _refuse_bf16_lengths(eng)
        lib.lv_lstm_bwd_len_f32(dh_ext, dh_last, mask, scale, whh, P(w.gates), P(w.hs), P(w.cs), P(w.dG), P(w.dGsum), P(w.lstm_ws),
                                dh0, dc0, tanh_init, P(steps[0]), steps[1], T, B, H, s)
        return
    if eng.precision != "bf16":
        lib.lv_lstm_bwd_f32(dh_ext, dh_last, mask, scale, whh, P(w.gates), P(w.hs), P(w.cs), P(w.dG), P(w.dGsum), P(w.lstm_ws),
                            dh0, dc0, tanh_init, T, B, H, s)
        return
    dG = P(w.dG) if img is None else None
    dG16 = P(img.dG) if img is not None else None
    if _persistent_ok(eng, img, B, H, device, _PERSIST_BWD_MAX_B):
        wi = eng._wimg
        rows = _persist_rows(eng, B)
        if mask is not None:
            raise _lib.LvaeError("the persistent BPTT has no in-kernel dropout mask (the engine applies it on dO)")
        if getattr(w, "saved_layout", None) != ("persist16", T, B, rows):
            raise _lib.LvaeError("the saved activations were not written by a persistent forward with the same T, B and rows per "
                                 "group (%r): eng.persist_rows / eng.persistent changed between forward and backward" % (getattr(w, "saved_layout", None),))
        lib.lv_lstm_bwd_bf16_persist16(dh_ext, dh_last, P(wi.bwd16), P(w.gates), P(w.hs), P(w.cs), dG16, P(w.dGsum), P(wi.xch),
                                       P(eng.status), dh0, dc0, tanh_init, T, B, rows, eng.persist_flags | _xch_flags(wi, "g", rows, device, T), H, s)
    else:
        _need_canonical_saved(w)
        lib.lv_lstm_bwd_bf16_img(dh_ext, dh_last, mask, scale, whh, P(w.gates), P(w.hs), P(w.cs), dG, dG16, P(w.dGsum),
                                 P(w.lstm_ws), dh0, dc0, tanh_init, T, B, H, s)


DUAL_WGRAD = os.environ.get("LVAE_DUAL_WGRAD", "1") != "0"
PAIR_WGRAD = os.environ.get("LVAE_PAIR_WGRAD", "1") != "0"
HS3_CVT = os.environ.get("LVAE_HS3_CVT", "1") != "0"


class _LstmImages(object):

    def __init__(self, c, TB, ni, H, key=None):
        self.TB, self.ni, self.H = TB, ni, H
        self.key = key
        self.ldr = _round_up(TB, 8)
        self.X = c.i16(TB, ni)
        self.XhT = c.i16(ni + H, self.ldr)
        self.addend = None
        self.dG = c.i16(TB, 4 * H)
        self.hT_gen = None
        self.hT_ld = self.ldr

    @property
    def XT(self):
        return self.XhT[:self.ni]

    @property
    def hT(self):
        return self.XhT[self.ni:]

    @staticmethod
    def usable(precision, native16, ni, H):
        return precision == "bf16" and native16 and ni % 8 == 0 and H % 8 == 0

    def forward(self, lib, s, X, W16, Gx, add_a, add_b, rows, wsc, addend_um=None, gather=None, h16=False, product=True):
        TB, ni, H = self.TB, self.ni, self.H
        if addend_um is not None:
            addend = addend_um
        else:
            if self.addend is None or self.addend.shape[0] != rows:
                self.addend = wsc.f32(rows, 4 * H)
                if self.key is not None:
                    wsc.grew(self.key, rows * 4 * H * 4)
            lib.lv_gate_interleave_f32(add_a, add_b, rows, H, P(self.addend), s)
            addend = P(self.addend)
        if h16:
            emb, ids, ids_stride, keep, kscale, T, B, V = gather
            assert keep is None
            lib.lv_cvt_h16_f32(emb, ni, TB, ni, 0, ids, ids_stride, B, V, P(self.X), ni, P(self.XT), self.ldr, s)
            if not product:
                return addend, 4 * H if rows > 1 else 0
            ws = _gemm_ws(lib, s)
            with _prof("gemm_bf16", 2.0 * TB * 4 * H * ni):
                lib.lv_gemm_h16(TB, 4 * H, ni, 1.0, P(self.X), ni, W16, ni, Gx, 4 * H, 0, addend, 4 * H if rows > 1 else 0, rows, None, 0, 1,
                                P(ws), ws.numel(), s)
            return
        if gather is not None:
            emb, ids, ids_stride, keep, kscale, T, B, V = gather
            lib.lv_embed_gather_b16(emb, ids, ids_stride, keep, kscale, T, B, ni, V, P(self.X), ni, P(self.XT), self.ldr, s)
        else:
            lib.lv_cvt_bf16_f32(X, ni, TB, ni, P(self.X), ni, P(self.XT), self.ldr, s)
        if not product:
            return addend, 4 * H if rows > 1 else 0
        _gemm16(lib, s, 0, TB, 4 * H, ni, P(self.X), ni, W16, ni, Gx, 4 * H,
                add1=addend, ld1=4 * H if rows > 1 else 0, mod1=rows)

    def backward(self, lib, s, dG, h_prev, WT16, dX, gW_ih, ld_gw, gW_hh, ws=None, between=None, hT_current=False):
        TB, ni, H = self.TB, self.ni, self.H
        if dG is not None:
            lib.lv_cvt_bf16_f32(dG, 4 * H, TB, 4 * H, P(self.dG), 4 * H, None, 0, s)
        wsd = ws if ws is not None else _gemm_ws(lib, s)
        if PAIR_WGRAD and DUAL_WGRAD and lib.lv_gemm_b16_pair_supported(1, 4 * H, ni + H, TB, 0, TB, ni, 4 * H, wsd.numel()):
            if not hT_current:
                lib.lv_cvt_bf16_f32(h_prev, H, TB, H, None, 0, P(self.hT), self.ldr, s)
            with _prof("gemm_bf16", 2.0 * 4 * H * (ni + H) * TB + 2.0 * TB * ni * 4 * H):
                lib.lv_gemm_b16_pair(1, 4 * H, ni + H, TB, P(self.dG), 4 * H, P(self.XhT), self.ldr, gW_ih, ld_gw, ni, gW_hh, H,
                                     0, TB, ni, 4 * H, P(self.dG), 4 * H, WT16, 4 * H, dX, ni, P(wsd), wsd.numel(), s)
            if between is not None:
                between()
            return
        _gemm16(lib, s, 0, TB, ni, 4 * H, P(self.dG), 4 * H, WT16, 4 * H, dX, ni, ws=ws)
        if between is not None:
            between()
        if not hT_current:
            lib.lv_cvt_bf16_f32(h_prev, H, TB, H, None, 0, P(self.hT), self.ldr, s)
        if DUAL_WGRAD and ni % 4 == 0 and lib.lv_gemm_b16_dual_supported(4 * H, ni + H, TB, wsd.numel()):
            with _prof("gemm_bf16", 2.0 * 4 * H * (ni + H) * TB):
                lib.lv_gemm_b16_dual(1, 4 * H, ni + H, TB, P(self.dG), 4 * H, P(self.XhT), self.ldr, gW_ih, ld_gw, ni, gW_hh, H,
                                     P(wsd), wsd.numel(), s)
            return
        _gemm16(lib, s, 1, 4 * H, ni, TB, P(self.dG), 4 * H, P(self.XT), self.ldr, gW_ih, ld_gw, ws=ws)
        _gemm16(lib, s, 1, 4 * H, H, TB, P(self.dG), 4 * H, P(self.hT), self.ldr, gW_hh, H, ws=ws)


class _LstmImagesMS(object):

    def __init__(self, c, Td, B, ns, ni, H):
        self.Td, self.B, self.ns, self.ni, self.H = Td, B, ns, ni, H
        self.TB, self.TBd = Td * B, Td * B * ns
        self.ldr, self.ldrd = _round_up(self.TB, 8), _round_up(self.TBd, 8)
        self.X = c.i16(self.TB, ni)
        self.XT = c.i16(ni, self.ldr)
        self.hT = c.i16(H, self.ldrd)
        self.dG = c.i16(self.TBd, 4 * H)
        self.dGs = c.i16(self.TB, 4 * H)
        self.hT_gen = None
        self.hT_ld = self.ldrd

    def forward(self, lib, s, W16, Gxw, gather):
        emb, ids, ids_stride, keep, kscale, T, B, V = gather
# ... 92 lines not shown
        persist = self.persistent and H == _PERSIST_H and B <= _PERSIST_MAX_B and torch.device(device).type == "cuda" and \
            torch.cuda.get_device_properties(device).multi_processor_count >= 256
        return _weight_images(self, self.lib, stream_ptr(device), device, persist)

    def ensure(self, device):
        device = torch.device(device)
        if self.flat is None or self.flat.device != device or not self.flat.bound():
            named = [("embed.weight", self.m.embed.weight), ("lstm.weight_ih_l0", self.m.lstm.weight_ih_l0),
                     ("lstm.weight_hh_l0", self.m.lstm.weight_hh_l0), ("lstm.bias_ih_l0", self.m.lstm.bias_ih_l0),
                     ("lstm.bias_hh_l0", self.m.lstm.bias_hh_l0), ("linear.weight", self.m.linear.weight)]
            self.flat = FlatBuffer(named, device)
            self.flat.flat_grads = getattr(self, "_flat_grads_pref", True)
            self.wsc = _WS(device)
            self.wsc.evictable = self.ws_evictable
            self.wsc.before_evict = self._quiesce_side_streams
            self._wimg = None
            for p in self.flat.params:
                p._lvae_engine = self
        self.lib = backend_for(device)
        if self.status is None or self.status.device != device:
            self.status = torch.zeros(1, dtype=torch.int32, device=device)
        return self.flat

    def dims(self):
        V, ni = self.m.embed.weight.shape
        H = self.m.lstm.weight_hh_l0.shape[1]
        nz2 = self.m.linear.weight.shape[0]
        return V, ni, H, nz2

    def _ws(self, B, T):
        V, ni, H, nz2 = self.dims()
        c = self.wsc

        def build():
            w = _NS()
            w.X = c.f32(T * B, ni)
            w.Gx, w.ws_key = None, (B, T)
            w.hs = torch.zeros(T + 1, B, H, dtype=torch.float32, device=c.device)
            w.cs = torch.zeros(T + 1, B, H, dtype=torch.float32, device=c.device)
            w.gates = c.f32(_saved_floats(self, T, B, H))
            w.mulv = c.f32(B, nz2)
            w.dmulv = c.f32(B, nz2)
            w.dG = c.f32(T * B, 4 * H)
            w.dGsum = c.f32(B, 4 * H)
            w.lstm_ws = c.f32(self.lib.lv_lstm_ws_floats(B, H))
            w.dhT = c.f32(B, H)
            w.dX = c.f32(T * B, ni)
            w.srows = c.i32(T * B)
            w.stok = c.i32(T * B)
            w.stmp = c.i32(2 * T * B)
            return w
        return c.get((B, T), build)

    def forward(self, x, head=None, x_key=None, lengths=None):
        assert x.dtype == torch.int64 and x.dim() == 2
        x = x.contiguous()
        B, T = x.shape
        steps = None
        if lengths is not None:
            _refuse_bf16_lengths(self)
            if head is not None:
                raise _lib.LvaeError("the fused head takes equal-length batches only")
            lengths = SeqLengths.of(lengths, B, T, x.device)
            steps = (lengths.enc, lengths.max)
        f = self.ensure(x.device)
        lib, s = self.lib, stream_ptr(x.device)
        V, ni, H, nz2 = self.dims()
        w = self._ws(B, T)
        v = f.views
        img = self._b16(B, T)
        exact = self._exact(img)
        self._h16_now = img is not None and not exact and self.fwd_operands == "f16"
        split = (self.exact_impl == "auto" and set(exact) == {"gx", "rec"} and _persistent_ok(self, img, B, H, x.device, _PERSIST_MAX_B))
        if img is None or ("gx" in exact and not split):
            lib.lv_embed_gather_f32(P(v["embed.weight"]), P(x), T, None, 1.0, P(w.X), T, B, ni, V, s)
        self._sort = _sorted_tokens(self, lib, s, x, x_key, T, T, B, V, w)
        biases = dict(add1=P(v["lstm.bias_ih_l0"]), ld1=0, mod1=1, add2=P(v["lstm.bias_hh_l0"]), ld2=0, mod2=1)
        gx_unit_major = True
        xin = None
        fuse_gx = (img is not None and not exact and steps is None and getattr(self, "gx_round", None) is None
                   and _fused_gx_ok(self, img, B, H, ni, x.device, FUSED_GX_ENC))
        if not fuse_gx:
            _gx_buffer(self.wsc, w, T * B, H)
        if split:
            self._exact_forward_split(lib, s, img, w, x, T, B, V, ni, H)
        elif img is not None and "gx" in exact:
            self.refresh_weight_images(B, x.device)
            lib.lv_embed_gather_b16(P(v["embed.weight"]), P(x), T, None, 1.0, T, B, ni, V, P(img.X), ni, P(img.XT), img.ldr, s)
            _gemm(lib, s, 0, 1, T * B, 4 * H, ni, P(w.X), ni, P(v["lstm.weight_ih_l0"]), ni, P(w.Gx), 4 * H, prec="f32", **biases)
            gx_unit_major = False
            if "rec" not in exact:
                if getattr(w, "Gx_gm", None) is None:
                    w.Gx_gm = self.wsc.f32(T * B, 4 * H)
                w.Gx, w.Gx_gm = w.Gx_gm, w.Gx
                lib.lv_gate_interleave_f32(P(w.Gx_gm), None, T * B, H, P(w.Gx), s)
                gx_unit_major = True
        elif img is not None:
            wi = self.refresh_weight_images(B, x.device)
            xin = img.forward(lib, s, None, P(wi.W), None if fuse_gx else P(w.Gx), P(v["lstm.bias_ih_l0"]), P(v["lstm.bias_hh_l0"]), 1,
                              self.wsc, gather=(P(v["embed.weight"]), P(x), T, None, 1.0, T, B, V), h16=self._h16_now, product=not fuse_gx)
        else:
            _gemm(lib, s, 0, 1, T * B, 4 * H, ni, P(w.X), ni, P(v["lstm.weight_ih_l0"]), ni, P(w.Gx), 4 * H,
                  prec=self.precision, **biases)
        gx_round = getattr(self, "gx_round", None)
        if gx_round is not None and not split:
            w.Gx.copy_(w.Gx.to(torch.float16 if gx_round == "f16" else torch.bfloat16).to(torch.float32))
        if split:
            pass
        elif "rec" in exact:
            self._exact_recurrence(lib, s, img, w, gx_unit_major, T, B, H, x.device)
        else:
            with _prof("lstm_fwd_enc", float(T), 1 if _persistent_ok(self, img, B, H, x.device, _PERSIST_MAX_B) else T):
                _lstm_forward(self, lib, s, img, w, None if fuse_gx else P(w.Gx), P(v["lstm.weight_hh_l0"]), None, 1.0, None, T, B, H,
                              x.device, steps=steps, xin=xin)
        if head is not None and not fused_ends_ok(B, nz2 // 2, head[0].shape[1]):
            eps, z, kl = head
            _gemm(lib, s, 0, 1, B, nz2, H, P(w.hs, T * B * H), H, P(v["linear.weight"]), H, P(w.mulv), nz2)
            lib.lv_reparam_kl_fwd_f32(P(w.mulv), P(eps), P(z), P(kl), B, eps.shape[1], nz2 // 2, s)
        elif head is not None:
            eps, z, kl = head
            lib.lv_enc_head_fwd_f32(P(w.hs, T * B * H), P(v["linear.weight"]), P(eps), P(w.mulv), P(z), P(kl), B, H,
                                    eps.shape[1], nz2 // 2, s)
        else:
            _gemm(lib, s, 0, 1, B, nz2, H, P(w.hs, T * B * H), H, P(v["linear.weight"]), H, P(w.mulv), nz2)
        self.gen += 1
        self.last = (x, B, T, self.gen)
        self.last_steps = steps
        return w.mulv

    def _exact_forward_split(self, lib, s, img, w, x, T, B, V, ni, H):
        v = self.flat.views
        TB = T * B
        wi = self.refresh_weight_images(B, x.device)
        c = self.wsc
        if getattr(wi, "Ww", None) is None:
            wi.Ww = c.i16(4 * H, 3 * ni)
            wi.Whh_lo = c.i16(4 * H, H)
        wih, whh = v["lstm.weight_ih_l0"], v["lstm.weight_hh_l0"]
        lib.lv_cvt_bf16_gates_f32(P(wih), wih.shape[1], H, ni, P(wi.Ww), 3 * ni, None, 0, s)
        lib.lv_cvt_bf16_gates_f32(P(wih), wih.shape[1], H, ni, P(wi.Ww, ni), 3 * ni, None, 0, s)
        lib.lv_cvt_bf16_lo_f32(P(wih), wih.shape[1], 4 * H, ni, H, None, 0, 1, 0, P(wi.Ww, 2 * ni), 3 * ni, None, 0, s)
        lib.lv_cvt_bf16_lo_f32(P(whh), H, 4 * H, H, H, None, 0, 1, 0, P(wi.Whh_lo), H, None, 0, s)
        if getattr(img, "Xw", None) is None:
            img.Xw = c.i16(TB, 3 * ni)
            img.h16 = c.i16(TB, H)
            if img.key is not None:
                c.grew(img.key, TB * (3 * ni + H) * 2)
        emb = P(v["embed.weight"])
        lib.lv_embed_gather_b16(emb, P(x), T, None, 1.0, T, B, ni, V, P(img.Xw), 3 * ni, P(img.XT), img.ldr, s)
        lib.lv_cvt_bf16_lo_f32(emb, ni, TB, ni, 0, P(x), T, B, V, P(img.Xw, ni), 3 * ni, None, 0, s)
        lib.lv_embed_gather_b16(emb, P(x), T, None, 1.0, T, B, ni, V, P(img.Xw, 2 * ni), 3 * ni, None, 0, s)
        if img.addend is None or img.addend.shape[0] != 1:
            img.addend = c.f32(1, 4 * H)
        lib.lv_gate_interleave_f32(P(v["lstm.bias_ih_l0"]), P(v["lstm.bias_hh_l0"]), 1, H, P(img.addend), s)
        _gemm16(lib, s, 0, TB, 4 * H, 3 * ni, P(img.Xw), 3 * ni, P(wi.Ww), 3 * ni, P(w.Gx), 4 * H, add1=P(img.addend), ld1=0, mod1=1)
        with _prof("lstm_fwd_enc", float(T), 1):
            _lstm_forward(self, lib, s, img, w, P(w.Gx), P(whh), None, 1.0, None, T, B, H, x.device)
        lib.lv_cvt_bf16_f32(P(w.hs), H, TB, H, P(img.h16), H, None, 0, s)
        _gemm16(lib, s, 0, TB, 4 * H, H, P(img.h16), H, P(wi.Whh_lo), H, P(w.Gx), 4 * H, acc=1)
        with _prof("lstm_fwd_enc", float(T), 1):
            _lstm_forward(self, lib, s, img, w, P(w.Gx), P(whh), None, 1.0, None, T, B, H, x.device)

    def _exact_recurrence(self, lib, s, img, w, gx_unit_major, T, B, H, device):
        v = self.flat.views
        n = T * B * 4 * H
        if getattr(w, "gates_canon", None) is None or w.gates_canon.numel() < n:
            w.gates_canon = self.wsc.f32(n)
        fwd = lib.lv_lstm_fwd_f32_ug if gx_unit_major else lib.lv_lstm_fwd_f32
        persist_bwd = _persistent_ok(self, img, B, H, device, _PERSIST_BWD_MAX_B)
        gates = w.gates_canon if persist_bwd else w.gates
        with _prof("lstm_fwd_enc", float(T), T):
            fwd(P(w.Gx), P(v["lstm.weight_hh_l0"]), P(w.hs), P(w.cs), P(gates), None, 1.0, None, P(w.lstm_ws), T, B, H, s)
        w.saved_layout = ("canonical", T, B, 0)
        if persist_bwd:
            rows = _persist_rows(self, B)
            need = lib.lv_lstm_persist16_saved_floats(T, rows)
            if w.gates.numel() < need:
# ... 22 lines not shown
        if head is not None:
            head = head[:4]
        if gate is not None and not (gate.dtype == torch.float32 and gate.is_contiguous() and tuple(gate.shape) == (B, nz2 // 2)):
            raise _lib.LvaeError("free-bits gate: a contiguous float32 [%d][%d] tensor expected" % (B, nz2 // 2))
        if iw and not fused_ends_ok(B, nz2 // 2, head[0].shape[1]):
            raise _lib.LvaeError("objective 'iw' runs on the one-launch encoder head (lv_enc_head_iw_bwd_f32); B = %d, nsamples = %d, "
                                 "nz = %d is beyond its LDS budget" % (B, head[0].shape[1], nz2 // 2))
        if head is not None and not fused_ends_ok(B, nz2 // 2, head[0].shape[1]):
            eps, dz, parts, dkl = head
            assert parts == 1
            if gate is not None:
                lib.lv_reparam_kl_gated_bwd_f32(P(w.mulv), P(eps), P(dz), P(dkl), P(gate), P(w.dmulv), B, eps.shape[1], nz2 // 2, s)
            else:
                lib.lv_reparam_kl_bwd_f32(P(w.mulv), P(eps), P(dz), P(dkl), P(w.dmulv), B, eps.shape[1], nz2 // 2, s)
            _gemm(lib, s, 0, 0, B, H, nz2, P(w.dmulv), nz2, P(v["linear.weight"]), H, P(w.dhT), H)
            _gemm(lib, s, 1, 0, nz2, H, B, P(w.dmulv), nz2, P(w.hs, T * B * H), H, P(gv["linear.weight"]), H)
        elif head is not None:
            eps, dz, parts, dkl = head
            if gate is not None:
                lib.lv_enc_head_gated_bwd_f32(P(w.mulv), P(eps), P(dz), parts, P(dkl), P(gate), P(w.hs, T * B * H), P(v["linear.weight"]),
                                              P(w.dmulv), P(w.dhT), P(gv["linear.weight"]), B, H, eps.shape[1], nz2 // 2, s)
            elif rs is not None:
                lib.lv_enc_head_dreg_bwd_f32(P(w.mulv), P(eps), P(dz), parts, P(dkl), P(rs), P(w.hs, T * B * H), P(v["linear.weight"]),
                                             P(w.dmulv), P(w.dhT), P(gv["linear.weight"]), B, H, eps.shape[1], nz2 // 2, s)
            else:
                head_bwd = lib.lv_enc_head_iw_bwd_f32 if iw else lib.lv_enc_head_bwd_f32
                head_bwd(P(w.mulv), P(eps), P(dz), parts, P(dkl), P(w.hs, T * B * H), P(v["linear.weight"]), P(w.dmulv),
                         P(w.dhT), P(gv["linear.weight"]), B, H, eps.shape[1], nz2 // 2, s)
        else:
            dmulv = dmulv.contiguous()
            _gemm(lib, s, 0, 0, B, H, nz2, P(dmulv), nz2, P(v["linear.weight"]), H, P(w.dhT), H)
            _gemm(lib, s, 1, 0, nz2, H, B, P(dmulv), nz2, P(w.hs, T * B * H), H, P(gv["linear.weight"]), H)
        img = self._b16(B, T)
        with _prof("lstm_bwd_enc", float(T), 1 if _persistent_ok(self, img, B, H, x.device, _PERSIST_BWD_MAX_B) else 2 * T):
            _lstm_backward(self, lib, s, img, w, None, P(w.dhT), None, 1.0, P(v["lstm.weight_hh_l0"]), None, None, 0, T, B, H, x.device,
                           steps=getattr(self, "last_steps", None))
        if after_bptt is not None:
            after_bptt()
        def embed_grad():
            self._aux.join(x.device)
            self.embed_rows = (self._sort[1], T * B)
            if self.fold and "embed" in self.fold:
                sq, only = self.fold["embed"]
                if only:
                    self.embed_rows = None
                lib.lv_embed_scatter_full_sumsq_f32(P(w.dX), None, 1.0, P(self._sort[0]), P(self._sort[1]), T, B, P(gv["embed.weight"]), ni,
                                                    V, -1, P(sq), int(only), s)
            else:
                lib.lv_embed_scatter_full_f32(P(w.dX), None, 1.0, P(self._sort[0]), P(self._sort[1]), T, B, P(gv["embed.weight"]), ni, V, -1, s)
            if after_embed is not None:
                after_embed()
        if img is not None:
            img.backward(lib, s, None, P(w.hs), P(self._wimg.WT), P(w.dX), P(gv["lstm.weight_ih_l0"]), ni, P(gv["lstm.weight_hh_l0"]),
                         between=embed_grad)
        else:
            _gemm(lib, s, 0, 0, T * B, ni, 4 * H, P(w.dG), 4 * H, P(v["lstm.weight_ih_l0"]), ni, P(w.dX), ni, prec=self.precision)
            embed_grad()
            _wgrad(lib, s, 4 * H, ni, T * B, P(w.dG), 4 * H, P(w.X), ni, P(gv["lstm.weight_ih_l0"]), ni, self.precision)
            _wgrad(lib, s, 4 * H, H, T * B, P(w.dG), 4 * H, P(w.hs), H, P(gv["lstm.weight_hh_l0"]), H, self.precision)
        lib.lv_colsum_f32(P(w.dGsum), 4 * H, B, 4 * H, P(gv["lstm.bias_ih_l0"]), P(gv["lstm.bias_hh_l0"]), s)


class LSTMDecoderEngine(object):

    def __init__(self, module):
        self.m = module
        self.flat = None
        self.wsc = None
        self.ws_evictable = True
        self.gen = 0
        self.precision = "f32"
        self.overlap = None
        self.native16 = True
        self.persistent = _PERSISTENT_DEFAULT
        self.persist_rows = None
        self.persist_flags = 1
        self.status = None
        self.fold = None
        self.cache_weight_images = True
        self.fused_nll = True
        self.wgen = 0
        self._wimg = None
        self._side = None
        self._side_ws = None
        self._pending = None
        self._aux = _AuxStream()
        self._sorts = _TokenSortCache()

    def _quiesce_side_streams(self):
        dev = self.flat.device if self.flat is not None else None
        if dev is not None and dev.type == "cuda":
            for st in (self._aux.stream, self._side):
                if st is not None:
                    torch.cuda.current_stream(dev).wait_stream(st)

    def _fork(self, device):
        import contextlib
        if not (torch.device(device).type == "cuda" and self._overlap_on()):
            return contextlib.nullcontext(), None
        if self._side is None:
            self._side = torch.cuda.Stream(device)
            self._side_ws = torch.empty(1 << 26, dtype=torch.float32, device=device)
        ev = torch.cuda.Event()
        ev.record(torch.cuda.current_stream(device))
        self._side.wait_event(ev)
        return torch.cuda.stream(self._side), self._side_ws

# ... 87 lines not shown
        return c.get(key, build)

    def fold_parts(self, B, Td, ns=1):
        out = {"embed": self.lib.lv_embed_scatter_sumsq_parts(Td, B)}
        V, ni, H, nz = self.dims()
        if self._b16(B * ns, Td, ns) is not None:
            dev = self.flat.device
            on_side = torch.device(dev).type == "cuda" and self._overlap_on()
            ws_n = (1 << 26) if on_side else _gemm_ws(self.lib, stream_ptr(dev)).numel()
            n = self.lib.lv_gemm_b16_sumsq_parts(V, H, Td * B * ns, ws_n)
            if n > 0:
                out["pred"] = n
        return out

    def _b16(self, Bd, Td, ns=1):
        V, ni, H, nz = self.dims()
        if self.precision != "bf16" or not self.native16 or H % 8 != 0:
            return None
        c = self.wsc

        def build():
            b = _NS()
            b.ldr = _round_up(Td * Bd, 8)
            b.ldv = _round_up(V, 32)
            b.O = c.i16(Td * Bd, H)
            b.OT = c.i16(H, b.ldr)
            b.dl = c.i16(Td * Bd, b.ldv)
            b.l16 = c.i16(Td * Bd, b.ldv)
            b.nparts = self.lib.lv_gemm_b16_nll_parts(V)
            b.part = c.f32(Td * Bd, 2 * b.nparts)
            b.tgt = c.f32(Td * Bd)
            return b
        return c.get(("b16", Bd, Td) if ns == 1 else ("b16", Bd // ns, ns, Td), build)

    def refresh_weight_images(self, B, device):
        V, ni, H, nz = self.dims()
        use_pred = self.precision == "bf16" and self.native16 and H % 8 == 0
        use_lstm = _LstmImages.usable(self.precision, self.native16, ni, H)
        if not (use_pred or use_lstm):
            return None
        self.ensure(device)
        persist = use_lstm and self.persistent and H == _PERSIST_H and B <= _PERSIST_MAX_B and \
            torch.device(device).type == "cuda" and torch.cuda.get_device_properties(device).multi_processor_count >= 256
        return _weight_images(self, self.lib, stream_ptr(device), device, persist, lstm=use_lstm, pred=use_pred)

    def _lstm_images(self, Bd, Td, ns=1):
        V, ni, H, nz = self.dims()
        if not _LstmImages.usable(self.precision, self.native16, ni, H):
            return None
        if ns > 1:
            return self.wsc.get(("b16lstm", Bd // ns, ns, Td), lambda: _LstmImagesMS(self.wsc, Td, Bd // ns, ns, ni, H))
        return self.wsc.get(("b16lstm", Bd, Td), lambda: _LstmImages(self.wsc, Td * Bd, ni, H, key=("b16lstm", Bd, Td)))

    def forward(self, x, z, mask_in, mask_out, p_in, p_out, want_rec=True, x_key=None, lengths=None):
        assert x.dtype == torch.int64 and x.dim() == 2
        x = x.contiguous()
        B, T = x.shape
        Td = T - 1
        if z.dim() != 3 or z.shape[0] != B or z.shape[1] < 1:
            raise _lib.LvaeError("the HIP decoder path takes z of shape [B, nsamples, nz]; got %s for a batch of %d" % (tuple(z.shape), B))
        ns = int(z.shape[1])
        Bd = B * ns
        steps = None
        if lengths is not None:
            _refuse_bf16_lengths(self)
            _same_device("the length-aware decoder", x.device, z=z, mask_in=mask_in, mask_out=mask_out)
            lengths = SeqLengths.of(lengths, B, T, x.device)
            steps = (lengths.dec(ns), lengths.max - 1)
        z2 = z.reshape(Bd, -1).contiguous()
        f = self.ensure(x.device)
        lib, s = self.lib, stream_ptr(x.device)
        V, ni, H, nz = self.dims()
        w = self._ws(Bd, Td, ns)
        v = f.views
        sc_in = 1.0 / (1.0 - p_in) if mask_in is not None else 1.0
        sc_out = 1.0 / (1.0 - p_out) if mask_out is not None else 1.0
        if mask_in is not None:
            assert mask_in.dtype == torch.uint8 and tuple(mask_in.shape) == (B, Td, ni) and mask_in.is_contiguous()
        if mask_out is not None:
            assert mask_out.dtype == torch.uint8 and tuple(mask_out.shape) == (Bd, Td, H) and mask_out.is_contiguous()
        gather = (P(v["embed.weight"]), P(x), T, P(mask_in), sc_in, Td, B, V)
        img = self._lstm_images(Bd, Td, ns)
        if img is None:
            lib.lv_embed_gather_f32(P(v["embed.weight"]), P(x), T, P(mask_in), sc_in, P(w.X), Td, B, ni, V, s)
        self._sort = _sorted_tokens(self, lib, s, x, x_key, T, Td, B, V, w)
        ids = x
        if ns > 1:
            lib.lv_repeat_rows_i64(P(x), P(w.x_rep), B, T, ns, s)
            ids = w.x_rep
        wih = v["lstm.weight_ih_l0"]
        fused = fused_ends_ok(Bd, nz)
        if fused:
            lib.lv_dec_init_f32(P(z2), P(v["trans_linear.weight"]), P(wih), ni + nz, ni, P(v["lstm.bias_ih_l0"]),
                                P(v["lstm.bias_hh_l0"]), P(w.cs), P(w.hs), P(w.Zp), 1 if img is not None else 0, Bd, H, nz, s)
        else:
            _gemm(lib, s, 0, 1, Bd, H, nz, P(z2), nz, P(v["trans_linear.weight"]), nz, P(w.cs), H)
            lib.lv_tanh_f32(P(w.cs), P(w.hs), Bd * H, s)
            _gemm(lib, s, 0, 1, Bd, 4 * H, nz, P(z2), nz, P(wih, ni), ni + nz, P(w.Zp), 4 * H,
                  add1=P(v["lstm.bias_ih_l0"]), ld1=0, mod1=1, add2=P(v["lstm.bias_hh_l0"]), ld2=0, mod2=1)
        xin = None
        fuse_gx = (ns == 1 and img is not None and steps is None and _fused_gx_ok(self, img, Bd, H, ni, x.device, FUSED_GX_DEC)
                   and self._b16(Bd, Td, ns) is not None)
        if not fuse_gx:
            _gx_buffer(self.wsc, w, Td * Bd, H)
        if ns > 1:
            zp = w.Zp
            if img is not None and not fused:
                lib.lv_gate_interleave_f32(P(w.Zp), None, Bd, H, P(w.Zp_um), s)
                zp = w.Zp_um
            if img is not None:
                wi = self.refresh_weight_images(Bd, x.device)
                img.forward(lib, s, P(wi.W), P(w.Gxw), gather)
            else:
                _gemm(lib, s, 0, 1, Td * B, 4 * H, ni, P(w.X), ni, P(wih), ni + nz, P(w.Gxw), 4 * H, prec=self.precision)
            lib.lv_gx_expand_add_f32(P(w.Gxw), P(zp), P(w.Gx), Td, B, ns, 4 * H, s)
        elif img is not None:
            wi = self.refresh_weight_images(B, x.device)
            gxp = None if fuse_gx else P(w.Gx)
            if fused:
                xin = img.forward(lib, s, None, P(wi.W), gxp, None, None, B, self.wsc, addend_um=P(w.Zp), gather=gather, product=not fuse_gx)
            else:
                xin = img.forward(lib, s, None, P(wi.W), gxp, P(w.Zp), None, B, self.wsc, gather=gather, product=not fuse_gx)
        else:
            _gemm(lib, s, 0, 1, Td * B, 4 * H, ni, P(w.X), ni, P(wih), ni + nz, P(w.Gx), 4 * H,
                  add1=P(w.Zp), ld1=4 * H, mod1=B, prec=self.precision)
        b16 = self._b16(Bd, Td, ns)
        late_mask = b16 is not None and _persistent_ok(self, img, Bd, H, x.device, _PERSIST_MAX_B)
        with _prof("lstm_fwd_dec", float(Td), 1 if _persistent_ok(self, img, Bd, H, x.device, _PERSIST_MAX_B) else Td):
            if late_mask:
                _lstm_forward(self, lib, s, img, w, None if fuse_gx else P(w.Gx), P(v["lstm.weight_hh_l0"]), None, 1.0, None, Td, Bd, H,
                              x.device, xin=xin)
            else:
                _lstm_forward(self, lib, s, img, w, P(w.Gx), P(v["lstm.weight_hh_l0"]), P(mask_out), sc_out, P(w.O), Td, Bd, H, x.device,
                              steps=steps)
        hs3 = HS3_CVT and late_mask and img is not None
        if hs3:
            lib.lv_cvt_bf16_hs3_f32(P(w.hs), H, Td, Bd, H, P(mask_out), sc_out, P(b16.O), H, P(b16.OT), b16.ldr, P(img.hT), img.hT_ld, s)
        if b16 is not None:
            if hs3:
                pass
            elif late_mask and mask_out is not None:
                lib.lv_cvt_bf16_keep_f32(P(w.hs, Bd * H), H, Td, Bd, H, P(mask_out), sc_out, P(b16.O), H, P(b16.OT), b16.ldr, s)
            elif late_mask:
                lib.lv_cvt_bf16_f32(P(w.hs, Bd * H), H, Td * Bd, H, P(b16.O), H, P(b16.OT), b16.ldr, s)
            else:
                lib.lv_cvt_bf16_f32(P(w.O), H, Td * Bd, H, P(b16.O), H, P(b16.OT), b16.ldr, s)
            wi = self.refresh_weight_images(Bd, x.device)
            if self.fused_nll:
                with _prof("gemm_bf16", 2.0 * Td * Bd * V * H):
                    lib.lv_gemm_b16_nll(Td * Bd, V, H, P(b16.O), H, P(wi.pred), H, P(b16.l16), b16.ldv, P(ids), T, 1, Bd,
                                        P(b16.part), P(b16.tgt), s)
                lib.lv_softmax_nll_merge_f32(P(b16.part), b16.nparts, P(b16.tgt), P(w.lse), P(w.nll), Td * Bd, s)
            else:
                _gemm16(lib, s, 0, Td * Bd, V, H, P(b16.O), H, P(wi.pred), H, P(w.logits), w.ldl)
        else:
            _gemm(lib, s, 0, 1, Td * Bd, V, H, P(w.O), H, P(v["pred_linear.weight"]), H, P(w.logits), w.ldl, prec=self.precision)
        if not (b16 is not None and self.fused_nll):
            lib.lv_softmax_nll_fwd_f32(P(w.logits), w.ldl, P(ids), T, 1, P(w.lse), P(w.nll), Td, Bd, V, s)
        if steps is not None:
            lib.lv_nll_mask_len_f32(P(w.nll), P(steps[0]), steps[1], Td, Bd, s)
        if want_rec:
            lib.lv_vae_loss_f32(P(w.nll), P(w.klz), P(w.zero1), P(w.loss), P(w.rec), Td, Bd, s)
        self.gen += 1
        if img is not None:
            img.hT_gen = self.gen if hs3 else None
        self.last = (x, z2, mask_in, mask_out, sc_in, sc_out, B, T, self.gen)
        self.last_ns = ns
        self.last_steps = steps
        return w.rec

    def cond_ll_supported(self, T):
        V, ni, H, nz = self.dims()
        return bool(self.lib.lv_dec_cond_ll_f32_supported(V, ni, H, nz, int(T)))

    def cond_ll(self, x, z):
# ... 1078 lines not shown
```

vae_lagging_encoder_amd/trainer.py:

```python
import collections
import ctypes
import os

import numpy as np
import contextlib
import gc
import torch

from . import engine as _eng
from .engine import P



@contextlib.contextmanager
def _capture_graph(graph, stream):
    was_enabled = gc.isenabled()
    gc.disable()
    try:
        with torch.cuda.graph(graph, stream=stream):
            yield
    finally:
        if was_enabled:
            gc.enable()

# ... 246 lines not shown
    def _static_for(self, B, T, parts=1):
        key = (B, T) if parts == 1 else (B, T, parts)
        st = self.static.get(key)
        if st is not None:
            self.static.move_to_end(key)
        else:
            d = self.device
            V, ni, H, nz = self.dec.dims()
            ns = self.nsamples
            st = _Static()
            st.x = torch.zeros(B, T, dtype=torch.int64, device=d)
            st.eps = torch.zeros(B, ns, nz, dtype=torch.float32, device=d)
            st.m_in = torch.ones(B, T - 1, ni, dtype=torch.uint8, device=d)
            st.m_out = torch.ones(B * ns, T - 1, H, dtype=torch.uint8, device=d)
            st.z = torch.empty(B, ns, nz, dtype=torch.float32, device=d)
            st.kl = torch.empty(B, dtype=torch.float32, device=d)
            st.loss = torch.empty(B, dtype=torch.float32, device=d)
            st.rec = torch.empty(B, dtype=torch.float32, device=d)
            st.gl = torch.full((B,), 1.0 / (B * parts), dtype=torch.float32, device=d)
            st.rowscale = torch.empty(B * ns, dtype=torch.float32, device=d)
            st.dkl = torch.empty(B, dtype=torch.float32, device=d)
            if self.objective == "iw":
                st.wz = torch.empty(B, ns, dtype=torch.float32, device=d)
                st.logw = torch.empty(B, ns, dtype=torch.float32, device=d)
                if self.iw_estimator == "dreg":
                    st.rs = torch.empty(B, ns, dtype=torch.float32, device=d)
            if self.free_bits is not None:
                st.kl_obj = torch.empty(B, dtype=torch.float32, device=d)
                st.kl_gate = torch.empty(B, nz, dtype=torch.float32, device=d)
            st.dmulv = torch.empty(B, 2 * nz, dtype=torch.float32, device=d)
            st.graphs = {}
            st.x_key = None
            st.xin = st.x
            self.static[key] = st
            if not self.use_graph:
                while len(self.static) > STATIC_SHAPES:
                    self.static.popitem(last=False)
        return st

    def _fwd_bwd(self, st, draw):
        self._arm_fold()
        try:
            self._fwd_bwd_armed(st, draw)
        finally:
            self.enc.fold = self.dec.fold = None

    def _fwd_bwd_armed(self, st, draw):
        lib, s = self.lib, _eng.stream_ptr(self.device)
        B, T = st.x.shape
        dec = self.vae.decoder
        train = self.vae.training
        use_in = train and dec.dropout_in.p > 0
        use_out = train and dec.dropout_out.p > 0
        if draw:
            lib.lv_rng_noise_step(P(st.eps), st.eps.numel(), P(st.m_in) if use_in else None, st.m_in.numel(),
                                  1.0 - dec.dropout_in.p, P(st.m_out) if use_out else None, st.m_out.numel(),
                                  1.0 - dec.dropout_out.p, P(self.rng_state), 0, s)
        m_in = st.m_in if use_in else None
        m_out = st.m_out if use_out else None
        mulv = self.enc.forward(st.xin, head=(st.eps, st.z, st.kl), x_key=st.x_key)
        if self.free_bits is not None:
            lib.lv_kl_freebits_fwd_f32(P(mulv), self.free_bits, self._fb_mode, P(st.kl_obj), P(st.kl_gate), None, B, st.eps.shape[2], s)
        self.dec.forward(st.xin, st.z, m_in, m_out, dec.dropout_in.p, dec.dropout_out.p, want_rec=False, x_key=st.x_key)
        ns = self.nsamples
        w = self.dec._ws(B * ns, T - 1, ns)
        iw = self.objective == "iw"
        fb = self.free_bits is not None
        if fb:
            a = (P(w.nll), P(st.kl), P(st.kl_obj), self._s(0), P(st.gl), P(st.loss), P(st.rec), P(st.rowscale), P(st.dkl),
                 self._s(10), T - 1, B, ns)
            if draw:
                lib.lv_loss_assemble_fb_rng_f32(*a, P(self.rng_state), 1, s)
            else:
                lib.lv_loss_assemble_fb_f32(*a, s)
        elif iw:
            dreg = self.iw_estimator == "dreg"
            a = (P(w.nll), P(mulv), P(st.eps), P(st.z), P(st.kl), self._s(0), P(st.gl), P(st.loss), P(st.rec),
                 P(st.rowscale), P(st.wz)) + ((P(st.rs),) if dreg else ()) + (P(st.logw), self._s(10), T - 1, B, ns, st.eps.shape[2])
            if draw:
                (lib.lv_loss_assemble_dreg_rng_f32 if dreg else lib.lv_loss_assemble_iw_rng_f32)(*a, P(self.rng_state), 1, s)
            else:
                (lib.lv_loss_assemble_dreg_f32 if dreg else lib.lv_loss_assemble_iw_f32)(*a, s)
        elif ns > 1 and draw:
            lib.lv_loss_assemble_ns_rng_f32(P(w.nll), P(st.kl), self._s(0), P(st.gl), P(st.loss), P(st.rec), P(st.rowscale), P(st.dkl),
                                            self._s(10), T - 1, B, ns, P(self.rng_state), 1, s)
        elif ns > 1:
            lib.lv_loss_assemble_ns_f32(P(w.nll), P(st.kl), self._s(0), P(st.gl), P(st.loss), P(st.rec), P(st.rowscale), P(st.dkl),
                                        self._s(10), T - 1, B, ns, s)
        elif draw:
            lib.lv_loss_assemble_rng_f32(P(w.nll), P(st.kl), self._s(0), P(st.gl), P(st.loss), P(st.rec), P(st.rowscale), P(st.dkl),
                                         self._s(10), T - 1, B, P(self.rng_state), 1, s)
        else:
            lib.lv_loss_assemble_f32(P(w.nll), P(st.kl), self._s(0), P(st.gl), P(st.loss), P(st.rec), P(st.rowscale), P(st.dkl),
                                     self._s(10), T - 1, B, s)
        dzp, parts = self.dec.backward(st.rowscale, partial_dz=True)
        hook = bucket = None
        if self.grad_sync is not None and not self._capturing and self.grad_sync.active:
            ef = self.enc.flat
            align = 1024 if self.grad_sync.payload == "bf16" else 4
            n_emb = ef.offsets[ef.names[1]] // align * align
            if self.grad_sync.rows is not None:
                j = self._row_index.get(id(st.x_key))
                if j is None:
                    raise _eng._lib.LvaeError("row-list exchange is on, but this batch tensor was not among those given to "
                                              "enable_row_exchange()")
                def bucket():
                    self.grad_sync.start_encoder_rows(ef, j)
            elif n_emb >= self.BUCKET_MIN_ELEMS and n_emb > 0:
                def bucket():
                    self.grad_sync.start_encoder_bucket(ef, 0, n_emb)
        if self.grad_sync is not None and not self._capturing:
            def start():
                self.dec.join()
                self.grad_sync.start_decoder(self.dec.flat, self._update)
            if self._collective_after_bptt():
                hook = start
            else:
                start()
        head = (st.eps, dzp, parts, st.wz, "iw") if iw else (st.eps, dzp, parts, st.dkl)
        if iw and self.iw_estimator == "dreg":
            head = (st.eps, dzp, parts, st.wz, "dreg", st.rs)
        if fb:
            head = (st.eps, dzp, parts, st.dkl, st.kl_gate)
        self.enc.backward(None, head=head, after_bptt=hook, after_embed=bucket)
        self.dec.join()
        if self.grad_sync is not None and self.grad_sync.active:
            ef = self.enc.flat
            lib.lv_txn_guard_f32(_eng.status_ptr(self.enc), _eng.status_ptr(self.dec), P(ef.grad_padded, ef.guard_index), s)

    def _collective_after_bptt(self):
        return bool(self.enc.persistent and self.enc.precision == "bf16")

    def _clip_and_step(self, update, dec_ss=None, embed_rows=None):
        lib, s = self.lib, _eng.stream_ptr(self.device)
        ef, df = self.enc.flat, self.dec.flat
        dp = self.grad_sync is not None and self.grad_sync.active
        gate = (_eng.status_ptr(self.enc), _eng.status_ptr(self.dec), P(ef.grad_padded, ef.guard_index) if dp else None,
                self._s(8), self._s(5))
        if dec_ss is None and self._fold is not None:
            f = self._fold
            lib.lv_clip_norm2_fold_txn_f32(P(ef.grad, f.enc_off), ef.numel - f.enc_off, P(df.grad, f.dec_off), f.dec_end - f.dec_off,
                                           P(self.norm_ws), P(f.parts), f.n, self.clip, self._s(2), self._s(3), self._s(4), *gate, s)
        elif dec_ss is None:
            lib.lv_clip_norm2_txn_f32(P(ef.grad), ef.numel, P(df.grad), df.numel, P(self.norm_ws), self.clip, self._s(2), self._s(3),
                                      self._s(4), *gate, s)
        else:
            lib.lv_sumsq_f32(P(ef.grad), ef.numel, P(self.norm_ws), self._s(2), 0, s)
            lib.lv_sum_accum_f32(P(dec_ss), 1, self._s(2), s)
            lib.lv_clip_coef_txn_f32(self._s(2), self.clip, self._s(3), self._s(4), *gate, s)
        if self.optimizer == "adam":
            self._adam_step(update, ef, df)
        elif self.sgd_buf is not None:
            self._sgd_momentum_step(update, ef, df)
        elif update == "both":
            lib.lv_sgd_step_txn_f32(P(ef.data), P(ef.grad), ef.numel, self._s(1), self._s(3), 1, self._s(8), s)
            lib.lv_sgd_step_txn_f32(P(df.data), P(df.grad), df.numel, self._s(1), self._s(3), 1, self._s(8), s)
        else:
            a, b = (ef, df) if update == "encoder" else (df, ef)
            b_off, b_n = 0, b.numel
            if update == "encoder" and self._fold is not None and self.decoder_grads == "norm":
                b_off, b_n = self._fold.dec_off, self._fold.dec_end - self._fold.dec_off
            emb = "embed.weight"
            if ROWS_SGD and update == "encoder" and embed_rows is not None and ef.names[0] == emb and ef.offsets[emb] == 0:
                stok, n_tok = embed_rows
                V, ni = self.enc.dims()[:2]
                lib.lv_sgd_step_scale_rows_txn_f32(P(a.data), P(a.grad), a.numel, self._s(1), self._s(3), 1, P(b.grad, b_off), b_n,
                                                   self._s(8), 0, V, ni, P(stok), n_tok, s)
            else:
                lib.lv_sgd_step_scale_txn_f32(P(a.data), P(a.grad), a.numel, self._s(1), self._s(3), 1, P(b.grad, b_off), b_n, self._s(8), s)

    def _sgd_momentum_step(self, update, ef, df):
        lib, s = self.lib, _eng.stream_ptr(self.device)
        sides = {"enc": ef, "dec": df}

        def args(k):
            f = sides[k]
            return (P(f.data), P(f.grad), P(self.sgd_buf[k]), f.numel, self._s(1), self._s(3), self.momentum, 1)
        if update == "both":
            lib.lv_sgd_momentum_step_txn_f32(*args("enc"), self._s(8), s)
            lib.lv_sgd_momentum_step_txn_f32(*args("dec"), self._s(8), s)
            return
# ... 576 lines not shown
```

Baseline: 12060.

## Fuse encoder-head and mid-step glue kernels into single multi-role launches

Adds two grouped kernels that partition the block index range across independent small tasks. One handles weight bf16 conversion, recurrent weight packing, embedding gather and conversion, RNG noise generation and bias interleave. The other handles the encoder head (mu/logvar, reparameterisation, KL), the hidden-state transpose and the decoder embedding pregather. The point is to cut kernel launch count and idle gaps on the plain ELBO training route. In exchange the trainer and encoder/decoder need new route gating and staleness tracking (hT_gen, pregathered keys), which makes the code more complex and could go stale if those guards miss a case.

```diff
diff --git a/include/lvae.h b/include/lvae.h
--- a/include/lvae.h
+++ b/include/lvae.h
@@ -284,6 +284,19 @@
                       float keep_out, uint64_t* state_dev, uint64_t inc, void* stream);
 int lv_rng_bernoulli_f32(const float* p, float* out, long n, const uint64_t* state_dev, uint64_t substream,
                          void* stream);
+
+int lv_glue_enc_head(const float* wih, long ld_wih, int H, int ni, uint16_t* W16, long ldw, uint16_t* WT16, long ldwt, int h16,
+                     const float* whh, float* wpk_fwd, float* wpk_bwd,
+                     const float* emb, const int64_t* ids, long ids_stride, int T, int B, int V,
+                     uint16_t* X16, long ldx, uint16_t* XT16, long ldxt,
+                     const float* b_ih, const float* b_hh, float* addend,
+                     float* eps, long n_eps, uint8_t* mask_in, long n_in, float keep_in, uint8_t* mask_out, long n_out, float keep_out,
+                     uint64_t* state_dev, void* stream);
+int lv_glue_mid(const float* h_last, const float* wlin, const float* eps, float* mulv, float* z, float* kl,
+                int B, int H, int ns, int nz,
+                const float* hs, int TB, uint16_t* hT16, long ldh,
+                const float* emb, const int64_t* ids, long ids_stride, const uint8_t* keep, float kscale,
+                int Td, int Bd, int ni, int V, uint16_t* X16, long ldx, uint16_t* XT16, long ldxt, void* stream);
 
 int lv_gauss_logpdf_f32(const float* z, const float* mu, const float* logvar, float* out, int B, int ns, int nz, void* stream);
 int lv_logsumexp_rows_f32(const float* in, long ld, int R, int C, float add, float* out, void* stream);
diff --git a/vae_lagging_encoder_amd/_lib.py b/vae_lagging_encoder_amd/_lib.py
--- a/vae_lagging_encoder_amd/_lib.py
+++ b/vae_lagging_encoder_amd/_lib.py
@@ -40,6 +40,10 @@
     "lv_cvt_bf16_lo_f32": [_vp, _l, _i, _i, _i, _vp, _l, _i, _i, _vp, _l, _vp, _l, _vp],
     "lv_cvt_h16_f32": [_vp, _l, _i, _i, _i, _vp, _l, _i, _i, _vp, _l, _vp, _l, _vp],
     "lv_gate_interleave_f32": [_vp, _vp, _i, _i, _vp, _vp],
+    "lv_glue_mid": [_vp, _vp, _vp, _vp, _vp, _vp, _i, _i, _i, _i, _vp, _i, _vp, _l, _vp, _vp, _l, _vp, _f, _i, _i, _i, _i,
+                    _vp, _l, _vp, _l, _vp],
+    "lv_glue_enc_head": [_vp, _l, _i, _i, _vp, _l, _vp, _l, _i, _vp, _vp, _vp, _vp, _vp, _l, _i, _i, _i, _vp, _l, _vp, _l,
+                         _vp, _vp, _vp, _vp, _l, _vp, _l, _f, _vp, _l, _f, _vp, _vp],
     "lv_lstm_fwd_bf16_ug": [_vp, _vp, _vp, _vp, _vp, _vp, _f, _vp, _vp, _i, _i, _i, _vp],
     "lv_lstm_fwd_f32_ug": [_vp, _vp, _vp, _vp, _vp, _vp, _f, _vp, _vp, _i, _i, _i, _vp],
     "lv_loss_assemble_f32": [_vp, _vp, _vp, _vp, _vp, _vp, _vp, _vp, _vp, _i, _i, _vp],
diff --git a/vae_lagging_encoder_amd/csrc/lv_gemm_b16.hip b/vae_lagging_encoder_amd/csrc/lv_gemm_b16.hip
--- a/vae_lagging_encoder_amd/csrc/lv_gemm_b16.hip
+++ b/vae_lagging_encoder_amd/csrc/lv_gemm_b16.hip
@@ -2,6 +2,7 @@
 #define lv_trace_buf lv_trace_buf_gemm
 #endif
 #include "lv_device.h"
+#include "lv_glue_bodies.h"
 #if defined(LV_TRACE) && !defined(LV_EMU)
 __device__ unsigned long long* lv_trace_buf = nullptr;
 extern "C" int lv_trace_set_gemm(void* p) { return (int)hipMemcpyToSymbol(HIP_SYMBOL(lv_trace_buf), &p, sizeof(p)); }
@@ -1613,84 +1614,8 @@
                                                          int gate_H, const uint8_t* __restrict__ keep, float kscale, int Bsz,
                                                          const int64_t* __restrict__ gids, long gstride, int gV, int lo) {
     __shared__ __attribute__((aligned(8))) uint16_t tile[64][68];
-    const int t = (int)threadIdx.x;
-    const int r0 = (int)blockIdx.y * 64, c0 = (int)blockIdx.x * 64;
-    const int q = t >> 4, cl = t & 15;
-    const bool tb = keep || gids;
-    const int Tt = tb ? R / Bsz : 1;
-    int bb = tb ? (r0 + q) % Bsz : 0, tt = tb ? (r0 + q) / Bsz : 0;
-    const int gc = c0 + 4 * cl;
-    const int gcc = gc < C ? gc : C - 4;
-    int grs[4], bbs[4], tts[4];
-    long sr[4];
-#pragma unroll
-    for (int u = 0; u < 4; ++u) {
-        grs[u] = r0 + q + 16 * u;
-        bbs[u] = bb; tts[u] = tt;
-        if (tb) {
-            bb += 16;
-            while (bb >= Bsz) { bb -= Bsz; ++tt; }
-        }
-        sr[u] = grs[u] < R ? grs[u] : R - 1;
-    }
-    if (gids) {
-#pragma unroll
-        for (int u = 0; u < 4; ++u) sr[u] = gids[(long)bbs[u] * gstride + (grs[u] < R ? tts[u] : 0)];
-#pragma unroll
-        for (int u = 0; u < 4; ++u) sr[u] = sr[u] < 0 ? 0 : (sr[u] >= gV ? gV - 1 : sr[u]);
-    }
-    float4 v[4];
-    uint32_t kp[4] = {0u, 0u, 0u, 0u};
-#pragma unroll
-    for (int u = 0; u < 4; ++u) v[u] = *reinterpret_cast<const float4*>(src + sr[u] * lds_ + gcc);
-    if (keep) {
-#pragma unroll
-        for (int u = 0; u < 4; ++u)
-            kp[u] = *reinterpret_cast<const uint32_t*>(keep + ((long)bbs[u] * Tt + (grs[u] < R ? tts[u] : 0)) * C + gcc);
-    }
-#pragma unroll
-    for (int u = 0; u < 4; ++u) {
-        const int gr = grs[u];
-        uint16_t b[4] = {0, 0, 0, 0}, d[4] = {0, 0, 0, 0};
-        const bool in = gr < R && gc < C;
-        if (in) {
-            const float xs[4] = {v[u].x, v[u].y, v[u].z, v[u].w};
-#pragma unroll
-            for (int e = 0; e < 4; ++e) {
-                float x = xs[e];
-                if (keep) {
-                    const bool k = (kp[u] >> (8 * e)) & 0xFFu;
-                    if (gids) x = k ? x * kscale : 0.f;
-                    else x *= k ? kscale : 0.f;
-                }
-                b[e] = (uint16_t)lv_f32_to_bf16_bits(x);
-                if (lo == 1) b[e] = (uint16_t)lv_f32_to_bf16_bits(x - lv_bf16_bits_to_f32(b[e]));
-                d[e] = lo == 2 ? lv_f32_to_f16_bits(lv_sat_f16(x)) : b[e];
-            }
-            if (dst) {
-                const long dr = gate_H > 0 ? (long)(gr % gate_H) * 4 + gr / gate_H : gr;
-                *reinterpret_cast<uint2*>(dst + dr * ldd + gc) = make_uint2((uint32_t)d[0] | ((uint32_t)d[1] << 16), (uint32_t)d[2] | ((uint32_t)d[3] << 16));
-            }
-        }
-        *reinterpret_cast<uint2*>(&tile[q + 16 * u][4 * cl]) = make_uint2((uint32_t)b[0] | ((uint32_t)b[1] << 16), (uint32_t)b[2] | ((uint32_t)b[3] << 16));
-    }
-    if (!dstT) return;
-    __syncthreads();
-    const int rl = t & 15, gr = r0 + 4 * rl;
-#pragma unroll
-    for (int i = 0; i < 4; ++i) {
-        const int c = q + 16 * i, gct = c0 + c;
-        const uint16_t e0 = tile[4 * rl][c], e1 = tile[4 * rl + 1][c], e2 = tile[4 * rl + 2][c], e3 = tile[4 * rl + 3][c];
-        if (gct < C) {
-            uint16_t* o = dstT + (long)gct * ldt + gr;
-            if (gr + 3 < R) *reinterpret_cast<uint2*>(o) = make_uint2((uint32_t)e0 | ((uint32_t)e1 << 16), (uint32_t)e2 | ((uint32_t)e3 << 16));
-            else {
-                if (gr < R) o[0] = e0;
-                if (gr + 1 < R) o[1] = e1;
-                if (gr + 2 < R) o[2] = e2;
-            }
-        }
-    }
+    const lv_glue::CvtP p{src, lds_, R, C, dst, ldd, dstT, ldt, gate_H, keep, kscale, Bsz, gids, gstride, gV, lo};
+    lv_glue::cvt_b16_v4_body(p, (int)blockIdx.x, (int)blockIdx.y, tile);
 }
 
 __global__ __launch_bounds__(256) void cvt_b16_hs3_kernel(const float* __restrict__ src, long lds_, int T, int Bsz, int C,
@@ -1782,9 +1707,7 @@
 static void cvt_launch(void* stream, const float* src, long lds, int R, int C, uint16_t* dst, long ldd, uint16_t* dstT, long ldt, int gate_H,
                        const uint8_t* keep, float kscale, int Bsz, const int64_t* gids, long gstride, int gV, int lo) {
     const dim3 grid((unsigned)lv_cdiv(C, 64), (unsigned)lv_cdiv(R, 64)), block(256);
-    const bool v4 = C >= 4 && C % 4 == 0 && lds % 4 == 0 && (((uintptr_t)src) & 15) == 0 &&
-                    (!dst || (ldd % 4 == 0 && (((uintptr_t)dst) & 7) == 0)) && (!dstT || (ldt % 4 == 0 && (((uintptr_t)dstT) & 7) == 0)) &&
-                    (!keep || (((uintptr_t)keep) & 3) == 0);
+    const bool v4 = lv_glue::cvt_v4_ok(lv_glue::CvtP{src, lds, R, C, dst, ldd, dstT, ldt, gate_H, keep, kscale, Bsz, gids, gstride, gV, lo});
     if (v4) LV_LAUNCH(cvt_b16_v4_kernel, grid, block, 0, stream, src, lds, R, C, dst, ldd, dstT, ldt, gate_H, keep, kscale, Bsz, gids, gstride, gV, lo);
     else LV_LAUNCH(cvt_b16_kernel, grid, block, 0, stream, src, lds, R, C, dst, ldd, dstT, ldt, gate_H, keep, kscale, Bsz, gids, gstride, gV, lo);
 }
diff --git a/vae_lagging_encoder_amd/csrc/lv_glue.hip b/vae_lagging_encoder_amd/csrc/lv_glue.hip
--- /dev/null
+++ b/vae_lagging_encoder_amd/csrc/lv_glue.hip
@@ -0,0 +1,122 @@
+#include "lv_device.h"
+#include "lv_glue_bodies.h"
+
+namespace {
+
+using namespace lv_glue;
+
+struct EncHeadP {
+    unsigned end[5];
+    CvtP w; unsigned w_nbx;
+    const float* whh; uint4* wfwd; uint4* wbwd; int fwd_f16;
+    CvtP x; unsigned x_nbx;
+    NoiseP n;
+    const float* ba; const float* bb; long gn; int H; float* addend;
+};
+
+__global__ __launch_bounds__(256) void glue_enc_head_kernel(EncHeadP p) {
+    __shared__ __attribute__((aligned(16))) unsigned char lds[CVT_TILE_BYTES];
+    const unsigned bid = blockIdx.x;
+    if (bid < p.end[0]) {
+        cvt_b16_v4_body(p.w, (int)(bid % p.w_nbx), (int)(bid / p.w_nbx), reinterpret_cast<uint16_t (*)[68]>(lds));
+    } else if (bid < p.end[1]) {
+        pack_w_both16_body(p.whh, p.wfwd, p.wbwd, p.fwd_f16, bid - p.end[0]);
+    } else if (bid < p.end[2]) {
+        const unsigned v = bid - p.end[1];
+        cvt_b16_v4_body(p.x, (int)(v % p.x_nbx), (int)(v / p.x_nbx), reinterpret_cast<uint16_t (*)[68]>(lds));
+    } else if (bid < p.end[3]) {
+        rng_noise_step_body(p.n, bid - p.end[2]);
+    } else {
+        gate_interleave_body(p.ba, p.bb, p.gn, p.H, p.addend, bid - p.end[3]);
+    }
+}
+
+constexpr int MID_LDS_BYTES = CVT_TILE_BYTES;
+struct MidP {
+    unsigned end[3];
+    const float* h_last; const float* wlin; const float* eps; float* mulv; float* z; float* kl; int H, ns, nz;
+    CvtP h; unsigned h_nbx;
+    CvtP x; unsigned x_nbx;
+};
+
+__global__ __launch_bounds__(256) void glue_mid_kernel(MidP p) {
+    __shared__ __attribute__((aligned(16))) unsigned char lds[MID_LDS_BYTES];
+    const unsigned bid = blockIdx.x;
+    if (bid < p.end[0]) {
+        enc_head_fwd_body(p.h_last, p.wlin, p.eps, p.mulv, p.z, p.kl, p.H, p.ns, p.nz, (int)bid, reinterpret_cast<char*>(lds));
+    } else if (bid < p.end[1]) {
+        const unsigned v = bid - p.end[0];
+        cvt_b16_v4_body(p.h, (int)(v % p.h_nbx), (int)(v / p.h_nbx), reinterpret_cast<uint16_t (*)[68]>(lds));
+    } else {
+        const unsigned v = bid - p.end[1];
+        cvt_b16_v4_body(p.x, (int)(v % p.x_nbx), (int)(v / p.x_nbx), reinterpret_cast<uint16_t (*)[68]>(lds));
+    }
+}
+
+}
+
+extern "C" int lv_glue_mid(const float* h_last, const float* wlin, const float* eps, float* mulv, float* z, float* kl,
+                           int B, int H, int ns, int nz,
+                           const float* hs, int TB, uint16_t* hT16, long ldh,
+                           const float* emb, const int64_t* ids, long ids_stride, const uint8_t* keep, float kscale,
+                           int Td, int Bd, int ni, int V, uint16_t* X16, long ldx, uint16_t* XT16, long ldxt, void* stream) {
+    if (!h_last || !wlin || !eps || !mulv || !z || !kl) return LV_ERR_ARG;
+    if (hs && !hT16) return LV_ERR_ARG;
+    if (emb && (!ids || !X16 || !XT16)) return LV_ERR_ARG;
+    if (B <= 0 || H <= 0 || ns <= 0 || nz <= 0) return LV_ERR_SHAPE;
+    if (hs && (TB <= 0 || ldh < TB)) return LV_ERR_SHAPE;
+    const long R = (long)Td * Bd;
+    if (emb && (Td <= 0 || Bd <= 0 || ni <= 0 || V <= 0 || R >= (1L << 31) || ldx < ni || ldxt < R)) return LV_ERR_SHAPE;
+    if ((size_t)(H + 3L * nz) * sizeof(float) > (size_t)MID_LDS_BYTES) return LV_ERR_UNSUPPORTED;
+    MidP p;
+    p.h_last = h_last; p.wlin = wlin; p.eps = eps; p.mulv = mulv; p.z = z; p.kl = kl; p.H = H; p.ns = ns; p.nz = nz;
+    p.h = CvtP{hs, (long)H, TB, H, nullptr, 0L, hT16, ldh, 0, nullptr, 1.f, 1, nullptr, 0L, 0, 0};
+    p.x = CvtP{emb, (long)ni, (int)R, ni, X16, ldx, XT16, ldxt, 0, keep, kscale, Bd, ids, ids_stride, V, 0};
+    if ((hs && !cvt_v4_ok(p.h)) || (emb && !cvt_v4_ok(p.x))) return LV_ERR_ALIGN;
+    p.h_nbx = (unsigned)lv_cdiv(H, 64);
+    p.x_nbx = emb ? (unsigned)lv_cdiv(ni, 64) : 1u;
+    p.end[0] = (unsigned)B;
+    p.end[1] = p.end[0] + (hs ? p.h_nbx * (unsigned)lv_cdiv(TB, 64) : 0u);
+    p.end[2] = p.end[1] + (emb ? p.x_nbx * (unsigned)lv_cdiv(R, 64) : 0u);
+    LV_LAUNCH(glue_mid_kernel, dim3(p.end[2]), dim3(256), 0, stream, p);
+    LV_CHECK_LAUNCH();
+    return LV_OK;
+}
+
+extern "C" int lv_glue_enc_head(const float* wih, long ld_wih, int H, int ni, uint16_t* W16, long ldw, uint16_t* WT16, long ldwt, int h16,
+                                const float* whh, float* wpk_fwd, float* wpk_bwd,
+                                const float* emb, const int64_t* ids, long ids_stride, int T, int B, int V,
+                                uint16_t* X16, long ldx, uint16_t* XT16, long ldxt,
+                                const float* b_ih, const float* b_hh, float* addend,
+                                float* eps, long n_eps, uint8_t* m_in, long n_in, float keep_in, uint8_t* m_out, long n_out, float keep_out,
+                                uint64_t* state, void* stream) {
+    if (!emb || !ids || !X16 || !XT16 || !b_ih || !addend) return LV_ERR_ARG;
+    if (wih && (!W16 || !WT16)) return LV_ERR_ARG;
+    if (whh && (!wpk_fwd || !wpk_bwd)) return LV_ERR_ARG;
+    if (eps && (!state || n_eps < 0 || n_in < 0 || n_out < 0)) return LV_ERR_ARG;
+    const long R = (long)T * B;
+    if (T <= 0 || B <= 0 || H <= 0 || ni <= 0 || V <= 0 || R >= (1L << 31) || ldx < ni || ldxt < R) return LV_ERR_SHAPE;
+    if (wih && (ld_wih < ni || ldw < ni || ldwt < 4L * H)) return LV_ERR_SHAPE;
+    if (whh && H != lvp::PH) return LV_ERR_UNSUPPORTED;
+    if (whh && ((((uintptr_t)wpk_fwd) | ((uintptr_t)wpk_bwd)) & 15) != 0) return LV_ERR_ALIGN;
+    const int lo = h16 ? 2 : 0;
+    EncHeadP p;
+    p.w = CvtP{wih, ld_wih, 4 * H, ni, W16, ldw, WT16, ldwt, H, nullptr, 1.f, 1, nullptr, 0L, 0, lo};
+    p.x = CvtP{emb, (long)ni, (int)R, ni, X16, ldx, XT16, ldxt, 0, nullptr, 1.f, B, ids, ids_stride, V, lo};
+    if ((wih && !cvt_v4_ok(p.w)) || !cvt_v4_ok(p.x)) return LV_ERR_ALIGN;
+    p.w_nbx = p.x_nbx = (unsigned)lv_cdiv(ni, 64);
+    p.whh = whh; p.wfwd = reinterpret_cast<uint4*>(wpk_fwd); p.wbwd = reinterpret_cast<uint4*>(wpk_bwd); p.fwd_f16 = h16 ? 1 : 0;
+    if (!m_in) n_in = 0;
+    if (!m_out) n_out = 0;
+    p.n = NoiseP{eps, n_eps, m_in, n_in, keep_in, m_out, n_out, keep_out, state, 0,
+                 (unsigned)lv_cdiv((n_eps + 3) / 4, 256), (unsigned)lv_cdiv((n_in + 7) / 8, 256)};
+    p.ba = b_ih; p.bb = b_hh; p.gn = 4L * H; p.H = H; p.addend = addend;
+    p.end[0] = wih ? p.w_nbx * (unsigned)lv_cdiv(4L * H, 64) : 0u;
+    p.end[1] = p.end[0] + (whh ? PACK_W_BOTH_BLOCKS : 0u);
+    p.end[2] = p.end[1] + p.x_nbx * (unsigned)lv_cdiv(R, 64);
+    p.end[3] = p.end[2] + (eps ? noise_blocks(p.n) : 0u);
+    p.end[4] = p.end[3] + (unsigned)lv_cdiv(p.gn, 256);
+    LV_LAUNCH(glue_enc_head_kernel, dim3(p.end[4]), dim3(256), 0, stream, p);
+    LV_CHECK_LAUNCH();
+    return LV_OK;
+}
diff --git a/vae_lagging_encoder_amd/csrc/lv_glue_bodies.h b/vae_lagging_encoder_amd/csrc/lv_glue_bodies.h
--- /dev/null
+++ b/vae_lagging_encoder_amd/csrc/lv_glue_bodies.h
@@ -0,0 +1,295 @@
+#pragma once
+#include "lv_device.h"
+#include "lv_persist_common.h"
+
+namespace lv_glue {
+
+struct U4 { uint32_t x, y, z, w; };
+
+__device__ __forceinline__ void mulhilo(uint32_t a, uint32_t b, uint32_t& hi, uint32_t& lo) {
+    const uint64_t p = (uint64_t)a * (uint64_t)b;
+    hi = (uint32_t)(p >> 32);
+    lo = (uint32_t)p;
+}
+
+__device__ __forceinline__ U4 philox4x32_10(U4 c, uint32_t k0, uint32_t k1) {
+#pragma unroll
+    for (int r = 0; r < 10; ++r) {
+        uint32_t hi0, lo0, hi1, lo1;
+        mulhilo(0xD2511F53u, c.x, hi0, lo0);
+        mulhilo(0xCD9E8D57u, c.z, hi1, lo1);
+        U4 n;
+        n.x = hi1 ^ c.y ^ k0;
+        n.y = lo1;
+        n.z = hi0 ^ c.w ^ k1;
+        n.w = lo0;
+        c = n;
+        k0 += 0x9E3779B9u;
+        k1 += 0xBB67AE85u;
+    }
+    return c;
+}
+
+__device__ __forceinline__ U4 draw(const uint64_t* state, uint64_t substream, uint64_t i) {
+    const uint64_t seed = state[0], off = state[1];
+    U4 c;
+    c.x = (uint32_t)i;
+    c.y = (uint32_t)(i >> 32);
+    c.z = (uint32_t)off ^ (uint32_t)(substream << 20);
+    c.w = (uint32_t)(off >> 32) ^ (uint32_t)(substream >> 12);
+    return philox4x32_10(c, (uint32_t)seed, (uint32_t)(seed >> 32));
+}
+
+__device__ __forceinline__ float u01(uint32_t x) { return ((float)(x >> 8) + 0.5f) * (1.0f / 16777216.0f); }
+
+struct NoiseP {
+    float* eps; long n_eps;
+    uint8_t* m1; long n1; float keep1;
+    uint8_t* m2; long n2; float keep2;
+    uint64_t* state; uint64_t inc;
+    unsigned nb0, nb1;
+};
+
+static inline unsigned noise_blocks(const NoiseP& p) { return p.nb0 + p.nb1 + (unsigned)lv_cdiv((p.n2 + 7) / 8, 256); }
+
+__device__ __forceinline__ void rng_noise_step_body(const NoiseP& p, unsigned bid) {
+    const int tid = (int)threadIdx.x;
+    if (bid < p.nb0) {
+        const long i = (long)bid * 256 + tid;
+        if (i * 4 < p.n_eps) {
+            const U4 r = draw(p.state, 0, (uint64_t)i);
+            const float u1 = u01(r.x), u2 = u01(r.y), u3 = u01(r.z), u4 = u01(r.w);
+            const float r1 = sqrtf(-2.f * logf(u1)), r2 = sqrtf(-2.f * logf(u3));
+            const float t1 = 6.283185307179586f * u2, t2 = 6.283185307179586f * u4;
+            const float v[4] = {r1 * cosf(t1), r1 * sinf(t1), r2 * cosf(t2), r2 * sinf(t2)};
+            for (int j = 0; j < 4; ++j)
+                if (i * 4 + j < p.n_eps) p.eps[i * 4 + j] = v[j];
+        }
+    } else {
+        const bool first = bid < p.nb0 + p.nb1;
+        uint8_t* out = first ? p.m1 : p.m2;
+        const long n = first ? p.n1 : p.n2;
+        const long i = (long)(bid - p.nb0 - (first ? 0u : p.nb1)) * 256 + tid;
+        if (i * 8 < n) {
+            const U4 r = draw(p.state, first ? 1 : 2, (uint64_t)i);
+            const uint32_t thr = (uint32_t)((first ? p.keep1 : p.keep2) * 65536.0f);
+            const uint32_t w[4] = {r.x, r.y, r.z, r.w};
+            if (i * 8 + 8 <= n && ((((uintptr_t)out) & 7) == 0)) {
+                uint32_t lo = 0, hi = 0;
+                for (int j = 0; j < 4; ++j) {
+                    lo |= (((w[j >> 1] >> ((j & 1) * 16)) & 0xFFFFu) < thr ? 1u : 0u) << (8 * j);
+                    hi |= (((w[2 + (j >> 1)] >> ((j & 1) * 16)) & 0xFFFFu) < thr ? 1u : 0u) << (8 * j);
+                }
+                *reinterpret_cast<uint2*>(out + i * 8) = make_uint2(lo, hi);
+            } else {
+                for (int j = 0; j < 8; ++j) {
+                    const uint32_t h = (w[j >> 1] >> ((j & 1) * 16)) & 0xFFFFu;
+                    if (i * 8 + j < n) out[i * 8 + j] = (h < thr) ? 1 : 0;
+                }
+            }
+        }
+    }
+}
+
+struct CvtP {
+    const float* src; long lds; int R, C;
+    uint16_t* dst; long ldd; uint16_t* dstT; long ldt;
+    int gate_H; const uint8_t* keep; float kscale; int Bsz;
+    const int64_t* gids; long gstride; int gV; int lo;
+};
+constexpr int CVT_TILE_BYTES = 64 * 68 * 2;
+
+static inline bool cvt_v4_ok(const CvtP& p) {
+    return p.C >= 4 && p.C % 4 == 0 && p.lds % 4 == 0 && (((uintptr_t)p.src) & 15) == 0 &&
+           (!p.dst || (p.ldd % 4 == 0 && (((uintptr_t)p.dst) & 7) == 0)) && (!p.dstT || (p.ldt % 4 == 0 && (((uintptr_t)p.dstT) & 7) == 0)) &&
+           (!p.keep || (((uintptr_t)p.keep) & 3) == 0);
+}
+
+__device__ __forceinline__ void cvt_b16_v4_body(const CvtP& p, int bx, int by, uint16_t (*tile)[68]) {
+    const float* __restrict__ src = p.src;
+    uint16_t* __restrict__ dst = p.dst;
+    uint16_t* __restrict__ dstT = p.dstT;
+    const uint8_t* __restrict__ keep = p.keep;
+    const int64_t* __restrict__ gids = p.gids;
+    const long lds_ = p.lds, ldd = p.ldd, ldt = p.ldt, gstride = p.gstride;
+    const int R = p.R, C = p.C, gate_H = p.gate_H, Bsz = p.Bsz, gV = p.gV, lo = p.lo;
+    const float kscale = p.kscale;
+    const int t = (int)threadIdx.x;
+    const int r0 = by * 64, c0 = bx * 64;
+    const int q = t >> 4, cl = t & 15;
+    const bool tb = keep || gids;
+    const int Tt = tb ? R / Bsz : 1;
+    int bb = tb ? (r0 + q) % Bsz : 0, tt = tb ? (r0 + q) / Bsz : 0;
+    const int gc = c0 + 4 * cl;
+    const int gcc = gc < C ? gc : C - 4;
+    int grs[4], bbs[4], tts[4];
+    long sr[4];
+#pragma unroll
+    for (int u = 0; u < 4; ++u) {
+        grs[u] = r0 + q + 16 * u;
+        bbs[u] = bb; tts[u] = tt;
+        if (tb) {
+            bb += 16;
+            while (bb >= Bsz) { bb -= Bsz; ++tt; }
+        }
+        sr[u] = grs[u] < R ? grs[u] : R - 1;
+    }
+    if (gids) {
+#pragma unroll
+        for (int u = 0; u < 4; ++u) sr[u] = gids[(long)bbs[u] * gstride + (grs[u] < R ? tts[u] : 0)];
+#pragma unroll
+        for (int u = 0; u < 4; ++u) sr[u] = sr[u] < 0 ? 0 : (sr[u] >= gV ? gV - 1 : sr[u]);
+    }
+    float4 v[4];
+    uint32_t kp[4] = {0u, 0u, 0u, 0u};
+#pragma unroll
+    for (int u = 0; u < 4; ++u) v[u] = *reinterpret_cast<const float4*>(src + sr[u] * lds_ + gcc);
+    if (keep) {
+#pragma unroll
+        for (int u = 0; u < 4; ++u)
+            kp[u] = *reinterpret_cast<const uint32_t*>(keep + ((long)bbs[u] * Tt + (grs[u] < R ? tts[u] : 0)) * C + gcc);
+    }
+#pragma unroll
+    for (int u = 0; u < 4; ++u) {
+        const int gr = grs[u];
+        uint16_t b[4] = {0, 0, 0, 0}, d[4] = {0, 0, 0, 0};
+        const bool in = gr < R && gc < C;
+        if (in) {
+            const float xs[4] = {v[u].x, v[u].y, v[u].z, v[u].w};
+#pragma unroll
+            for (int e = 0; e < 4; ++e) {
+                float x = xs[e];
+                if (keep) {
+                    const bool k = (kp[u] >> (8 * e)) & 0xFFu;
+                    if (gids) x = k ? x * kscale : 0.f;
+                    else x *= k ? kscale : 0.f;
+                }
+                b[e] = (uint16_t)lv_f32_to_bf16_bits(x);
+                if (lo == 1) b[e] = (uint16_t)lv_f32_to_bf16_bits(x - lv_bf16_bits_to_f32(b[e]));
+                d[e] = lo == 2 ? lv_f32_to_f16_bits(lv_sat_f16(x)) : b[e];
+            }
+            if (dst) {
+                const long dr = gate_H > 0 ? (long)(gr % gate_H) * 4 + gr / gate_H : gr;
+                *reinterpret_cast<uint2*>(dst + dr * ldd + gc) = make_uint2((uint32_t)d[0] | ((uint32_t)d[1] << 16), (uint32_t)d[2] | ((uint32_t)d[3] << 16));
+            }
+        }
+        *reinterpret_cast<uint2*>(&tile[q + 16 * u][4 * cl]) = make_uint2((uint32_t)b[0] | ((uint32_t)b[1] << 16), (uint32_t)b[2] | ((uint32_t)b[3] << 16));
+    }
+    if (!dstT) return;
+    __syncthreads();
+    const int rl = t & 15, gr = r0 + 4 * rl;
+#pragma unroll
+    for (int i = 0; i < 4; ++i) {
+        const int c = q + 16 * i, gct = c0 + c;
+        const uint16_t e0 = tile[4 * rl][c], e1 = tile[4 * rl + 1][c], e2 = tile[4 * rl + 2][c], e3 = tile[4 * rl + 3][c];
+        if (gct < C) {
+            uint16_t* o = dstT + (long)gct * ldt + gr;
+            if (gr + 3 < R) *reinterpret_cast<uint2*>(o) = make_uint2((uint32_t)e0 | ((uint32_t)e1 << 16), (uint32_t)e2 | ((uint32_t)e3 << 16));
+            else {
+                if (gr < R) o[0] = e0;
+                if (gr + 1 < R) o[1] = e1;
+                if (gr + 2 < R) o[2] = e2;
+            }
+        }
+    }
+}
+
+__device__ __forceinline__ void pack_w_k16_one(const float* __restrict__ whh, uint4* __restrict__ wpk, long idx, int f16 = 0) {
+    constexpr int PH = lvp::PH;
+    const int l = (int)(idx & 63), nb = (int)((idx >> 6) & 7), ks = (int)((idx >> 9) & 7);
+    const int wave_id = (int)(idx >> 12), m = wave_id >> 2, w = wave_id & 3;
+    const int c = l & 15, kq = l >> 4, col = 16 * nb + c;
+    const float* row = whh + ((long)(col & 3) * PH + 32 * m + (col >> 2)) * PH + 256 * w + 32 * ks + 8 * kq;
+    if (f16) {
+        float r[8];
+#pragma unroll
+        for (int e = 0; e < 8; ++e) r[e] = lv_sat_f16(row[e]);
+        wpk[idx] = make_uint4(lv_pack_f16x2(r[0], r[1]), lv_pack_f16x2(r[2], r[3]), lv_pack_f16x2(r[4], r[5]), lv_pack_f16x2(r[6], r[7]));
+    }
+    else
+        wpk[idx] = make_uint4(lv_pack_bf16x2(row[0], row[1]), lv_pack_bf16x2(row[2], row[3]), lv_pack_bf16x2(row[4], row[5]),
+                              lv_pack_bf16x2(row[6], row[7]));
+}
+__device__ __forceinline__ void pack_w_rs16_one(const float* __restrict__ whh, uint4* __restrict__ wpk, long idx) {
+    constexpr int PH = lvp::PH;
+    const int l = (int)(idx & 63), nb = (int)((idx >> 6) & 15), ks = (int)((idx >> 10) & 3);
+    const int wave_id = (int)(idx >> 12), m = wave_id >> 2, w = wave_id & 3;
+    const int c = l & 15, kq = l >> 4, j = 256 * w + 16 * nb + c;
+    float v[8];
+#pragma unroll
+    for (int e = 0; e < 8; ++e) {
+        const int n2 = 32 * ks + 8 * kq + e;
+        v[e] = whh[((long)(n2 & 3) * PH + 32 * m + (n2 >> 2)) * PH + j];
+    }
+    wpk[idx] = make_uint4(lv_pack_bf16x2(v[0], v[1]), lv_pack_bf16x2(v[2], v[3]), lv_pack_bf16x2(v[4], v[5]), lv_pack_bf16x2(v[6], v[7]));
+}
+constexpr long PACK_W_ONE = 128L * 64 * 64;
+constexpr unsigned PACK_W_BOTH_BLOCKS = (unsigned)(2 * PACK_W_ONE / 256);
+__device__ __forceinline__ void pack_w_both16_body(const float* __restrict__ whh, uint4* __restrict__ wfwd, uint4* __restrict__ wbwd,
+                                                   int fwd_f16, unsigned bid) {
+    const long n = PACK_W_ONE;
+    const long idx = (long)bid * 256 + threadIdx.x;
+    if (idx < n) pack_w_k16_one(whh, wfwd, idx, fwd_f16);
+    else if (idx < 2 * n) pack_w_rs16_one(whh, wbwd, idx - n);
+}
+
+__device__ __forceinline__ void gate_interleave_body(const float* __restrict__ a, const float* __restrict__ b, long n, int H,
+                                                     float* __restrict__ out, unsigned bid) {
+    const long idx = (long)bid * 256 + threadIdx.x;
+    if (idx >= n) return;
+    const long r = idx / (4L * H);
+    const int c = (int)(idx % (4L * H));
+    const long src = r * 4L * H + (long)(c & 3) * H + (c >> 2);
+    out[idx] = a[src] + (b ? b[src] : 0.f);
+}
+
+__device__ __forceinline__ void enc_head_fwd_body(const float* __restrict__ hT, const float* __restrict__ wlin,
+                                                  const float* __restrict__ eps, float* __restrict__ mulv,
+                                                  float* __restrict__ z, float* __restrict__ kl,
+                                                  int H, int ns, int nz, int b, char* smem) {
+    float* sh = reinterpret_cast<float*>(smem);
+    float* sm = sh + H;
+    float* sk = sm + 2 * nz;
+    const int tid = (int)threadIdx.x, l = tid & 63, w = tid >> 6;
+    const int nz2 = 2 * nz;
+    for (int h = tid; h < H; h += 256) sh[h] = hT[(long)b * H + h];
+    __syncthreads();
+    for (int o0 = 0; o0 < nz2; o0 += 64) {
+        float acc[16];
+#pragma unroll
+        for (int i = 0; i < 16; ++i) acc[i] = 0.f;
+#pragma unroll 4
+        for (int h = l; h < H; h += 64) {
+            const float x = sh[h];
+#pragma unroll
+            for (int i = 0; i < 16; ++i) {
+                const int o = o0 + w + 4 * i;
+                acc[i] = fmaf(x, wlin[(long)(o < nz2 ? o : 0) * H + h], acc[i]);
+            }
+        }
+#pragma unroll
+        for (int i = 0; i < 16; ++i) {
+            const int o = o0 + w + 4 * i;
+            const float s = lv_wave_sum(acc[i]);
+            if (l == 0 && o < nz2) { sm[o] = s; mulv[(long)b * nz2 + o] = s; }
+        }
+    }
+    __syncthreads();
+    for (int j = tid; j < nz; j += 256) {
+        const float m = sm[j], lv = sm[nz + j];
+        const float sd = expf(0.5f * lv);
+        sk[j] = (m * m + expf(lv)) - lv - 1.f;
+        for (int s = 0; s < ns; ++s) {
+            const long zi = ((long)b * ns + s) * nz + j;
+            z[zi] = m + eps[zi] * sd;
+        }
+    }
+    __syncthreads();
+    if (tid == 0) {
+        float s = 0.f;
+        for (int j = 0; j < nz; ++j) s += sk[j];
+        kl[b] = 0.5f * s;
+    }
+}
+
+}
diff --git a/vae_lagging_encoder_amd/csrc/lv_head.hip b/vae_lagging_encoder_amd/csrc/lv_head.hip
--- a/vae_lagging_encoder_amd/csrc/lv_head.hip
+++ b/vae_lagging_encoder_amd/csrc/lv_head.hip
@@ -1,4 +1,5 @@
 #include "lv_device.h"
+#include "lv_glue_bodies.h"
 
 namespace {
 
@@ -32,49 +33,7 @@
                                                            float* __restrict__ z, float* __restrict__ kl,
                                                            int H, int ns, int nz) {
     LV_DYN_SHARED(smem);
-    float* sh = reinterpret_cast<float*>(smem);
-    float* sm = sh + H;
-    float* sk = sm + 2 * nz;
-    const int b = (int)blockIdx.x, tid = (int)threadIdx.x, l = tid & 63, w = tid >> 6;
-    const int nz2 = 2 * nz;
-    for (int h = tid; h < H; h += 256) sh[h] = hT[(long)b * H + h];
-    __syncthreads();
-    for (int o0 = 0; o0 < nz2; o0 += 64) {
-        float acc[16];
-#pragma unroll
-        for (int i = 0; i < 16; ++i) acc[i] = 0.f;
-#pragma unroll 4
-        for (int h = l; h < H; h += 64) {
-            const float x = sh[h];
-#pragma unroll
-            for (int i = 0; i < 16; ++i) {
-                const int o = o0 + w + 4 * i;
-                acc[i] = fmaf(x, wlin[(long)(o < nz2 ? o : 0) * H + h], acc[i]);
-            }
-        }
-#pragma unroll
-        for (int i = 0; i < 16; ++i) {
-            const int o = o0 + w + 4 * i;
-            const float s = lv_wave_sum(acc[i]);
-            if (l == 0 && o < nz2) { sm[o] = s; mulv[(long)b * nz2 + o] = s; }
-        }
-    }
-    __syncthreads();
-    for (int j = tid; j < nz; j += 256) {
-        const float m = sm[j], lv = sm[nz + j];
-        const float sd = expf(0.5f * lv);
-        sk[j] = (m * m + expf(lv)) - lv - 1.f;
-        for (int s = 0; s < ns; ++s) {
-            const long zi = ((long)b * ns + s) * nz + j;
-            z[zi] = m + eps[zi] * sd;
-        }
-    }
-    __syncthreads();
-    if (tid == 0) {
-        float s = 0.f;
-        for (int j = 0; j < nz; ++j) s += sk[j];
-        kl[b] = 0.5f * s;
-    }
+    lv_glue::enc_head_fwd_body(hT, wlin, eps, mulv, z, kl, H, ns, nz, (int)blockIdx.x, smem);
 }
 
 __device__ __forceinline__ const float* head_gate(const float* g) { return g; }
diff --git a/vae_lagging_encoder_amd/csrc/lv_lstm.hip b/vae_lagging_encoder_amd/csrc/lv_lstm.hip
--- a/vae_lagging_encoder_amd/csrc/lv_lstm.hip
+++ b/vae_lagging_encoder_amd/csrc/lv_lstm.hip
@@ -1,4 +1,5 @@
 #include "lv_device.h"
+#include "lv_glue_bodies.h"
 
 namespace {
 
@@ -693,12 +694,7 @@
 namespace {
 __global__ __launch_bounds__(256) void gate_interleave_kernel(const float* __restrict__ a, const float* __restrict__ b,
                                                               long n, int H, float* __restrict__ out) {
-    const long idx = (long)blockIdx.x * 256 + threadIdx.x;
-    if (idx >= n) return;
-    const long r = idx / (4L * H);
-    const int c = (int)(idx % (4L * H));
-    const long src = r * 4L * H + (long)(c & 3) * H + (c >> 2);
-    out[idx] = a[src] + (b ? b[src] : 0.f);
+    lv_glue::gate_interleave_body(a, b, n, H, out, blockIdx.x);
 }
 }
 
diff --git a/vae_lagging_encoder_amd/csrc/lv_lstm_persist16.hip b/vae_lagging_encoder_amd/csrc/lv_lstm_persist16.hip
--- a/vae_lagging_encoder_amd/csrc/lv_lstm_persist16.hip
+++ b/vae_lagging_encoder_amd/csrc/lv_lstm_persist16.hip
@@ -1,5 +1,6 @@
 #include "lv_device.h"
 #include "lv_persist_common.h"
+#include "lv_glue_bodies.h"
 
 #if defined(LV_TRACE) && !defined(LV_EMU)
 __device__ unsigned long long* lv_trace_buf = nullptr;
@@ -29,39 +30,11 @@
 __global__ __launch_bounds__(256) void pack_w_k16_kernel(const float* __restrict__ whh, uint4* __restrict__ wpk, int f16);
 __global__ __launch_bounds__(256) void pack_w_rs16_kernel(const float* __restrict__ whh, uint4* __restrict__ wpk);
 
-__device__ __forceinline__ void pack_w_k16_one(const float* __restrict__ whh, uint4* __restrict__ wpk, long idx, int f16 = 0) {
-    const int l = (int)(idx & 63), nb = (int)((idx >> 6) & 7), ks = (int)((idx >> 9) & 7);
-    const int wave_id = (int)(idx >> 12), m = wave_id >> 2, w = wave_id & 3;
-    const int c = l & 15, kq = l >> 4, col = 16 * nb + c;
-    const float* row = whh + ((long)(col & 3) * PH + 32 * m + (col >> 2)) * PH + 256 * w + 32 * ks + 8 * kq;
-    if (f16) {
-        float r[8];
-#pragma unroll
-        for (int e = 0; e < 8; ++e) r[e] = lv_sat_f16(row[e]);
-        wpk[idx] = make_uint4(lv_pack_f16x2(r[0], r[1]), lv_pack_f16x2(r[2], r[3]), lv_pack_f16x2(r[4], r[5]), lv_pack_f16x2(r[6], r[7]));
-    }
-    else
-        wpk[idx] = make_uint4(lv_pack_bf16x2(row[0], row[1]), lv_pack_bf16x2(row[2], row[3]), lv_pack_bf16x2(row[4], row[5]),
-                              lv_pack_bf16x2(row[6], row[7]));
-}
-__device__ __forceinline__ void pack_w_rs16_one(const float* __restrict__ whh, uint4* __restrict__ wpk, long idx) {
-    const int l = (int)(idx & 63), nb = (int)((idx >> 6) & 15), ks = (int)((idx >> 10) & 3);
-    const int wave_id = (int)(idx >> 12), m = wave_id >> 2, w = wave_id & 3;
-    const int c = l & 15, kq = l >> 4, j = 256 * w + 16 * nb + c;
-    float v[8];
-#pragma unroll
-    for (int e = 0; e < 8; ++e) {
-        const int n2 = 32 * ks + 8 * kq + e;
-        v[e] = whh[((long)(n2 & 3) * PH + 32 * m + (n2 >> 2)) * PH + j];
-    }
-    wpk[idx] = make_uint4(lv_pack_bf16x2(v[0], v[1]), lv_pack_bf16x2(v[2], v[3]), lv_pack_bf16x2(v[4], v[5]), lv_pack_bf16x2(v[6], v[7]));
-}
+using lv_glue::pack_w_k16_one;
+using lv_glue::pack_w_rs16_one;
 __global__ __launch_bounds__(256) void pack_w_both16_kernel(const float* __restrict__ whh, uint4* __restrict__ wfwd, uint4* __restrict__ wbwd,
                                                             int fwd_f16) {
-    const long n = 128L * 64 * 64;
-    const long idx = (long)blockIdx.x * 256 + threadIdx.x;
-    if (idx < n) pack_w_k16_one(whh, wfwd, idx, fwd_f16);
-    else if (idx < 2 * n) pack_w_rs16_one(whh, wbwd, idx - n);
+    lv_glue::pack_w_both16_body(whh, wfwd, wbwd, fwd_f16, blockIdx.x);
 }
 
 __global__ __launch_bounds__(256) void pack_w_k16_kernel(const float* __restrict__ whh, uint4* __restrict__ wpk, int f16) {
diff --git a/vae_lagging_encoder_amd/csrc/lv_rng.hip b/vae_lagging_encoder_amd/csrc/lv_rng.hip
--- a/vae_lagging_encoder_amd/csrc/lv_rng.hip
+++ b/vae_lagging_encoder_amd/csrc/lv_rng.hip
@@ -1,44 +1,9 @@
 #include "lv_device.h"
+#include "lv_glue_bodies.h"
 
 namespace {
 
-struct U4 { uint32_t x, y, z, w; };
-
-__device__ __forceinline__ void mulhilo(uint32_t a, uint32_t b, uint32_t& hi, uint32_t& lo) {
-    const uint64_t p = (uint64_t)a * (uint64_t)b;
-    hi = (uint32_t)(p >> 32);
-    lo = (uint32_t)p;
-}
-
-__device__ __forceinline__ U4 philox4x32_10(U4 c, uint32_t k0, uint32_t k1) {
-#pragma unroll
-    for (int r = 0; r < 10; ++r) {
-        uint32_t hi0, lo0, hi1, lo1;
-        mulhilo(0xD2511F53u, c.x, hi0, lo0);
-        mulhilo(0xCD9E8D57u, c.z, hi1, lo1);
-        U4 n;
-        n.x = hi1 ^ c.y ^ k0;
-        n.y = lo1;
-        n.z = hi0 ^ c.w ^ k1;
-        n.w = lo0;
-        c = n;
-        k0 += 0x9E3779B9u;
-        k1 += 0xBB67AE85u;
-    }
-    return c;
-}
-
-__device__ __forceinline__ U4 draw(const uint64_t* state, uint64_t substream, uint64_t i) {
-    const uint64_t seed = state[0], off = state[1];
-    U4 c;
-    c.x = (uint32_t)i;
-    c.y = (uint32_t)(i >> 32);
-    c.z = (uint32_t)off ^ (uint32_t)(substream << 20);
-    c.w = (uint32_t)(off >> 32) ^ (uint32_t)(substream >> 12);
-    return philox4x32_10(c, (uint32_t)seed, (uint32_t)(seed >> 32));
-}
-
-__device__ __forceinline__ float u01(uint32_t x) { return ((float)(x >> 8) + 0.5f) * (1.0f / 16777216.0f); }
+using namespace lv_glue;
 
 __global__ __launch_bounds__(256) void rng_normal_kernel(float* __restrict__ out, long n, const uint64_t* __restrict__ state,
                                                          uint64_t substream) {
@@ -80,53 +45,7 @@
     if (threadIdx.x == 0 && blockIdx.x == 0) state[1] += inc;
 }
 
-struct NoiseP {
-    float* eps; long n_eps;
-    uint8_t* m1; long n1; float keep1;
-    uint8_t* m2; long n2; float keep2;
-    uint64_t* state; uint64_t inc;
-    unsigned nb0, nb1;
-};
-
-__global__ __launch_bounds__(256) void rng_noise_step_kernel(NoiseP p) {
-    const unsigned bid = blockIdx.x;
-    const int tid = (int)threadIdx.x;
-    if (bid < p.nb0) {
-        const long i = (long)bid * 256 + tid;
-        if (i * 4 < p.n_eps) {
-            const U4 r = draw(p.state, 0, (uint64_t)i);
-            const float u1 = u01(r.x), u2 = u01(r.y), u3 = u01(r.z), u4 = u01(r.w);
-            const float r1 = sqrtf(-2.f * logf(u1)), r2 = sqrtf(-2.f * logf(u3));
-            const float t1 = 6.283185307179586f * u2, t2 = 6.283185307179586f * u4;
-            const float v[4] = {r1 * cosf(t1), r1 * sinf(t1), r2 * cosf(t2), r2 * sinf(t2)};
-            for (int j = 0; j < 4; ++j)
-                if (i * 4 + j < p.n_eps) p.eps[i * 4 + j] = v[j];
-        }
-    } else {
-        const bool first = bid < p.nb0 + p.nb1;
-        uint8_t* out = first ? p.m1 : p.m2;
-        const long n = first ? p.n1 : p.n2;
-        const long i = (long)(bid - p.nb0 - (first ? 0u : p.nb1)) * 256 + tid;
-        if (i * 8 < n) {
-            const U4 r = draw(p.state, first ? 1 : 2, (uint64_t)i);
-            const uint32_t thr = (uint32_t)((first ? p.keep1 : p.keep2) * 65536.0f);
-            const uint32_t w[4] = {r.x, r.y, r.z, r.w};
-            if (i * 8 + 8 <= n && ((((uintptr_t)out) & 7) == 0)) {
-                uint32_t lo = 0, hi = 0;
-                for (int j = 0; j < 4; ++j) {
-                    lo |= (((w[j >> 1] >> ((j & 1) * 16)) & 0xFFFFu) < thr ? 1u : 0u) << (8 * j);
-                    hi |= (((w[2 + (j >> 1)] >> ((j & 1) * 16)) & 0xFFFFu) < thr ? 1u : 0u) << (8 * j);
-                }
-                *reinterpret_cast<uint2*>(out + i * 8) = make_uint2(lo, hi);
-            } else {
-                for (int j = 0; j < 8; ++j) {
-                    const uint32_t h = (w[j >> 1] >> ((j & 1) * 16)) & 0xFFFFu;
-                    if (i * 8 + j < n) out[i * 8 + j] = (h < thr) ? 1 : 0;
-                }
-            }
-        }
-    }
-}
+__global__ __launch_bounds__(256) void rng_noise_step_kernel(NoiseP p) { rng_noise_step_body(p, blockIdx.x); }
 
 }
 
@@ -171,7 +90,7 @@
     if (!mask_out) n_out = 0;
     NoiseP p{eps, n_eps, mask_in, n_in, keep_in, mask_out, n_out, keep_out, state, inc,
              (unsigned)lv_cdiv((n_eps + 3) / 4, 256), (unsigned)lv_cdiv((n_in + 7) / 8, 256)};
-    const unsigned nb = p.nb0 + p.nb1 + (unsigned)lv_cdiv((n_out + 7) / 8, 256);
+    const unsigned nb = noise_blocks(p);
     if (nb > 0) LV_LAUNCH(rng_noise_step_kernel, dim3(nb), dim3(256), 0, stream, p);
     if (inc != 0) LV_LAUNCH(rng_advance_kernel, dim3(1), dim3(64), 0, stream, state, inc);
     LV_CHECK_LAUNCH();
diff --git a/vae_lagging_encoder_amd/engine.py b/vae_lagging_encoder_amd/engine.py
--- a/vae_lagging_encoder_amd/engine.py
+++ b/vae_lagging_encoder_amd/engine.py
@@ -407,7 +407,7 @@
     return (sum(p._version for p in eng.flat.params), eng.wgen)
 
 
-def _weight_images(eng, lib, s, device, want_persist, lstm=True, pred=False):
+def _weight_images(eng, lib, s, device, want_persist, lstm=True, pred=False, defer=False):
     wi = eng._wimg
     V, ni, H = eng.dims()[:3]
     v = eng.flat.views
@@ -427,9 +427,13 @@
     ver = weights_version(eng) if eng.cache_weight_images else object()
     h16 = bool(getattr(eng, "_h16_now", False))
     stale = wi.ver != ver or getattr(wi, "h16", False) != h16
+    if defer:
+        assert wi.W is not None and wi.pred is None and want_persist
     if stale:
         wih = v["lstm.weight_ih_l0"]
-        if wi.W is not None and h16:
+        if defer:
+            pass
+        elif wi.W is not None and h16:
             lib.lv_cvt_h16_f32(P(wih), wih.shape[1], 4 * H, ni, H, None, 0, 1, 0, P(wi.W), ni, P(wi.WT), 4 * H, s)
         elif wi.W is not None:
             lib.lv_cvt_bf16_gates_f32(P(wih), wih.shape[1], H, ni, P(wi.W), ni, P(wi.WT), 4 * H, s)
@@ -438,13 +442,15 @@
             lib.lv_cvt_bf16_f32(P(v["pred_linear.weight"]), H, V, H, P(wi.pred), H, P(wi.predT), wi.ldv, s)
         wi.ver = ver
         wi.packed16 = False
+    wi.todo = (stale, bool(want_persist and not wi.packed16)) if defer else None
     if want_persist and not wi.packed16:
         if wi.fwd16 is None:
             n = lib.lv_lstm_persist16_wpk_floats()
             wi.fwd16, wi.bwd16 = c.f32(n), c.f32(n)
             wi.xch = torch.zeros(lib.lv_lstm_persist16_xch_floats(), dtype=torch.float32, device=c.device)
             wi.xstate = {"f": 0, "g": 0, "gcls": [0, 0]}
-        (lib.lv_lstm_persist16_pack2_h16 if h16 else lib.lv_lstm_persist16_pack2)(P(v["lstm.weight_hh_l0"]), P(wi.fwd16), P(wi.bwd16), H, s)
+        if not defer:
+            (lib.lv_lstm_persist16_pack2_h16 if h16 else lib.lv_lstm_persist16_pack2)(P(v["lstm.weight_hh_l0"]), P(wi.fwd16), P(wi.bwd16), H, s)
         wi.packed16 = True
     return wi
 
@@ -681,6 +687,9 @@
 PAIR_WGRAD = os.environ.get("LVAE_PAIR_WGRAD", "1") != "0"
 HS3_CVT = os.environ.get("LVAE_HS3_CVT", "1") != "0"
 
+GLUE_HEAD = os.environ.get("LVAE_GLUE_HEAD", "1") != "0"
+GLUE_MID = os.environ.get("LVAE_GLUE_MID", "1") != "0"
+
 
 class _LstmImages(object):
 
@@ -707,21 +716,30 @@
     def usable(precision, native16, ni, H):
         return precision == "bf16" and native16 and ni % 8 == 0 and H % 8 == 0
 
-    def forward(self, lib, s, X, W16, Gx, add_a, add_b, rows, wsc, addend_um=None, gather=None, h16=False, product=True):
+    def own_addend(self, wsc, rows):
+        if self.addend is None or self.addend.shape[0] != rows:
+            self.addend = wsc.f32(rows, 4 * self.H)
+            if self.key is not None:
+                wsc.grew(self.key, rows * 4 * self.H * 4)
+        return self.addend
+
+    def forward(self, lib, s, X, W16, Gx, add_a, add_b, rows, wsc, addend_um=None, gather=None, h16=False, product=True,
+                have_addend=False, have_images=False):
         TB, ni, H = self.TB, self.ni, self.H
         if addend_um is not None:
             addend = addend_um
         else:
-            if self.addend is None or self.addend.shape[0] != rows:
-                self.addend = wsc.f32(rows, 4 * H)
-                if self.key is not None:
-                    wsc.grew(self.key, rows * 4 * H * 4)
-            lib.lv_gate_interleave_f32(add_a, add_b, rows, H, P(self.addend), s)
+            self.own_addend(wsc, rows)
+            if not have_addend:
+                lib.lv_gate_interleave_f32(add_a, add_b, rows, H, P(self.addend), s)
             addend = P(self.addend)
+        if have_images:
+            assert gather is not None
         if h16:
             emb, ids, ids_stride, keep, kscale, T, B, V = gather
             assert keep is None
-            lib.lv_cvt_h16_f32(emb, ni, TB, ni, 0, ids, ids_stride, B, V, P(self.X), ni, P(self.XT), self.ldr, s)
+            if not have_images:
+                lib.lv_cvt_h16_f32(emb, ni, TB, ni, 0, ids, ids_stride, B, V, P(self.X), ni, P(self.XT), self.ldr, s)
             if not product:
                 return addend, 4 * H if rows > 1 else 0
             ws = _gemm_ws(lib, s)
@@ -729,7 +747,9 @@
                 lib.lv_gemm_h16(TB, 4 * H, ni, 1.0, P(self.X), ni, W16, ni, Gx, 4 * H, 0, addend, 4 * H if rows > 1 else 0, rows, None, 0, 1,
                                 P(ws), ws.numel(), s)
             return
-        if gather is not None:
+        if have_images:
+            pass
+        elif gather is not None:
             emb, ids, ids_stride, keep, kscale, T, B, V = gather
             lib.lv_embed_gather_b16(emb, ids, ids_stride, keep, kscale, T, B, ni, V, P(self.X), ni, P(self.XT), self.ldr, s)
         else:
@@ -928,7 +948,7 @@
             return w
         return c.get((B, T), build)
 
-    def forward(self, x, head=None, x_key=None, lengths=None):
+    def forward(self, x, head=None, x_key=None, lengths=None, glue=False, noise=None, mid=None):
         assert x.dtype == torch.int64 and x.dim() == 2
         x = x.contiguous()
         B, T = x.shape
@@ -948,6 +968,11 @@
         exact = self._exact(img)
         self._h16_now = img is not None and not exact and self.fwd_operands == "f16"
         split = (self.exact_impl == "auto" and set(exact) == {"gx", "rec"} and _persistent_ok(self, img, B, H, x.device, _PERSIST_MAX_B))
+        hT_gen = None
+        glue_head = (glue and GLUE_HEAD and img is not None and not exact and steps is None and ni % 4 == 0
+                     and _persistent_ok(self, img, B, H, x.device, _PERSIST_MAX_B))
+        if noise is not None and not glue_head:
+            lib.lv_rng_noise_step(*(noise + (0, s)))
         if img is None or ("gx" in exact and not split):
             lib.lv_embed_gather_f32(P(v["embed.weight"]), P(x), T, None, 1.0, P(w.X), T, B, ni, V, s)
         self._sort = _sorted_tokens(self, lib, s, x, x_key, T, T, B, V, w)
@@ -972,9 +997,20 @@
                 lib.lv_gate_interleave_f32(P(w.Gx_gm), None, T * B, H, P(w.Gx), s)
                 gx_unit_major = True
         elif img is not None:
-            wi = self.refresh_weight_images(B, x.device)
+            if glue_head:
+                wi = _weight_images(self, lib, s, x.device, True, defer=True)
+                wih, h16 = v["lstm.weight_ih_l0"], self._h16_now
+                stale_w, stale_pk = wi.todo
+                lib.lv_glue_enc_head(P(wih) if stale_w else None, wih.shape[1], H, ni, P(wi.W), ni, P(wi.WT), 4 * H, 1 if h16 else 0,
+                                     P(v["lstm.weight_hh_l0"]) if stale_pk else None, P(wi.fwd16), P(wi.bwd16),
+                                     P(v["embed.weight"]), P(x), T, T, B, V, P(img.X), ni, P(img.XT), img.ldr,
+                                     P(v["lstm.bias_ih_l0"]), P(v["lstm.bias_hh_l0"]), P(img.own_addend(self.wsc, 1)),
+                                     *((noise or (None, 0, None, 0, 1.0, None, 0, 1.0, None)) + (s,)))
+            else:
+                wi = self.refresh_weight_images(B, x.device)
             xin = img.forward(lib, s, None, P(wi.W), None if fuse_gx else P(w.Gx), P(v["lstm.bias_ih_l0"]), P(v["lstm.bias_hh_l0"]), 1,
-                              self.wsc, gather=(P(v["embed.weight"]), P(x), T, None, 1.0, T, B, V), h16=self._h16_now, product=not fuse_gx)
+                              self.wsc, gather=(P(v["embed.weight"]), P(x), T, None, 1.0, T, B, V), h16=self._h16_now, product=not fuse_gx,
+                              have_addend=glue_head, have_images=glue_head)
         else:
             _gemm(lib, s, 0, 1, T * B, 4 * H, ni, P(w.X), ni, P(v["lstm.weight_ih_l0"]), ni, P(w.Gx), 4 * H,
                   prec=self.precision, **biases)
@@ -995,10 +1031,17 @@
             lib.lv_reparam_kl_fwd_f32(P(w.mulv), P(eps), P(z), P(kl), B, eps.shape[1], nz2 // 2, s)
         elif head is not None:
             eps, z, kl = head
-            lib.lv_enc_head_fwd_f32(P(w.hs, T * B * H), P(v["linear.weight"]), P(eps), P(w.mulv), P(z), P(kl), B, H,
-                                    eps.shape[1], nz2 // 2, s)
+            hargs = (P(w.hs, T * B * H), P(v["linear.weight"]), P(eps), P(w.mulv), P(z), P(kl), B, H, eps.shape[1], nz2 // 2)
+            if (mid is not None and glue and GLUE_MID and img is not None and steps is None
+                    and _persistent_ok(self, img, B, H, x.device, _PERSIST_MAX_B) and (H + 3 * (nz2 // 2)) * 4 <= 8704):
+                mid(hargs + (P(w.hs), T * B, P(img.hT), img.ldr))
+                hT_gen = self.gen + 1
+            else:
+                lib.lv_enc_head_fwd_f32(*(hargs + (s,)))
         else:
             _gemm(lib, s, 0, 1, B, nz2, H, P(w.hs, T * B * H), H, P(v["linear.weight"]), H, P(w.mulv), nz2)
+        if img is not None:
+            img.hT_gen = hT_gen
         self.gen += 1
         self.last = (x, B, T, self.gen)
         self.last_steps = steps
@@ -1127,7 +1170,7 @@
                 after_embed()
         if img is not None:
             img.backward(lib, s, None, P(w.hs), P(self._wimg.WT), P(w.dX), P(gv["lstm.weight_ih_l0"]), ni, P(gv["lstm.weight_hh_l0"]),
-                         between=embed_grad)
+                         between=embed_grad, hT_current=img.hT_gen == g)
         else:
             _gemm(lib, s, 0, 0, T * B, ni, 4 * H, P(w.dG), 4 * H, P(v["lstm.weight_ih_l0"]), ni, P(w.dX), ni, prec=self.precision)
             embed_grad()
@@ -1321,6 +1364,19 @@
             return self.wsc.get(("b16lstm", Bd // ns, ns, Td), lambda: _LstmImagesMS(self.wsc, Td, Bd // ns, ns, ni, H))
         return self.wsc.get(("b16lstm", Bd, Td), lambda: _LstmImages(self.wsc, Td * Bd, ni, H, key=("b16lstm", Bd, Td)))
 
+    def pregather(self, x, mask_in, p_in):
+        assert x.dtype == torch.int64 and x.dim() == 2 and x.is_contiguous()
+        self._pregathered = None
+        B, T = x.shape
+        f = self.ensure(x.device)
+        V, ni, H, nz = self.dims()
+        img = self._lstm_images(B, T - 1, 1)
+        if img is None or T < 2 or ni % 4 != 0 or (mask_in is not None and mask_in.data_ptr() % 4 != 0):
+            return None
+        sc_in = 1.0 / (1.0 - p_in) if mask_in is not None else 1.0
+        self._pregathered = (x.data_ptr(), None if mask_in is None else mask_in.data_ptr(), sc_in, self.gen)
+        return (P(f.views["embed.weight"]), P(x), T, P(mask_in), sc_in, T - 1, B, ni, V, P(img.X), ni, P(img.XT), img.ldr)
+
     def forward(self, x, z, mask_in, mask_out, p_in, p_out, want_rec=True, x_key=None, lengths=None):
         assert x.dtype == torch.int64 and x.dim() == 2
         x = x.contiguous()
@@ -1349,6 +1405,9 @@
         if mask_out is not None:
             assert mask_out.dtype == torch.uint8 and tuple(mask_out.shape) == (Bd, Td, H) and mask_out.is_contiguous()
         gather = (P(v["embed.weight"]), P(x), T, P(mask_in), sc_in, Td, B, V)
+        pre, self._pregathered = getattr(self, "_pregathered", None), None
+        pre = (pre is not None and ns == 1 and steps is None
+               and pre == (x.data_ptr(), None if mask_in is None else mask_in.data_ptr(), sc_in, self.gen))
         img = self._lstm_images(Bd, Td, ns)
         if img is None:
             lib.lv_embed_gather_f32(P(v["embed.weight"]), P(x), T, P(mask_in), sc_in, P(w.X), Td, B, ni, V, s)
@@ -1387,9 +1446,11 @@
             wi = self.refresh_weight_images(B, x.device)
             gxp = None if fuse_gx else P(w.Gx)
             if fused:
-                xin = img.forward(lib, s, None, P(wi.W), gxp, None, None, B, self.wsc, addend_um=P(w.Zp), gather=gather, product=not fuse_gx)
+                xin = img.forward(lib, s, None, P(wi.W), gxp, None, None, B, self.wsc, addend_um=P(w.Zp), gather=gather, product=not fuse_gx,
+                                  have_images=pre)
             else:
-                xin = img.forward(lib, s, None, P(wi.W), gxp, P(w.Zp), None, B, self.wsc, gather=gather, product=not fuse_gx)
+                xin = img.forward(lib, s, None, P(wi.W), gxp, P(w.Zp), None, B, self.wsc, gather=gather, product=not fuse_gx,
+                                  have_images=pre)
         else:
             _gemm(lib, s, 0, 1, Td * B, 4 * H, ni, P(w.X), ni, P(wih), ni + nz, P(w.Gx), 4 * H,
                   add1=P(w.Zp), ld1=4 * H, mod1=B, prec=self.precision)
diff --git a/vae_lagging_encoder_amd/trainer.py b/vae_lagging_encoder_amd/trainer.py
--- a/vae_lagging_encoder_amd/trainer.py
+++ b/vae_lagging_encoder_amd/trainer.py
@@ -322,13 +322,20 @@
         train = self.vae.training
         use_in = train and dec.dropout_in.p > 0
         use_out = train and dec.dropout_out.p > 0
+        noise, glue = None, self._plain_route()
         if draw:
-            lib.lv_rng_noise_step(P(st.eps), st.eps.numel(), P(st.m_in) if use_in else None, st.m_in.numel(),
-                                  1.0 - dec.dropout_in.p, P(st.m_out) if use_out else None, st.m_out.numel(),
-                                  1.0 - dec.dropout_out.p, P(self.rng_state), 0, s)
+            noise = (P(st.eps), st.eps.numel(), P(st.m_in) if use_in else None, st.m_in.numel(),
+                     1.0 - dec.dropout_in.p, P(st.m_out) if use_out else None, st.m_out.numel(),
+                     1.0 - dec.dropout_out.p, P(self.rng_state))
+            if not glue:
+                lib.lv_rng_noise_step(*(noise + (0, s)))
+                noise = None
         m_in = st.m_in if use_in else None
         m_out = st.m_out if use_out else None
-        mulv = self.enc.forward(st.xin, head=(st.eps, st.z, st.kl), x_key=st.x_key)
+        def mid(enc_args):
+            ga = self.dec.pregather(st.xin, m_in, dec.dropout_in.p)
+            lib.lv_glue_mid(*(enc_args + (ga or (None, None, 0, None, 1.0, 0, 0, 0, 0, None, 0, None, 0)) + (s,)))
+        mulv = self.enc.forward(st.xin, head=(st.eps, st.z, st.kl), x_key=st.x_key, glue=glue, noise=noise, mid=mid if glue else None)
         if self.free_bits is not None:
             lib.lv_kl_freebits_fwd_f32(P(mulv), self.free_bits, self._fb_mode, P(st.kl_obj), P(st.kl_gate), None, B, st.eps.shape[2], s)
         self.dec.forward(st.xin, st.z, m_in, m_out, dec.dropout_in.p, dec.dropout_out.p, want_rec=False, x_key=st.x_key)
@@ -397,6 +404,10 @@
         if self.grad_sync is not None and self.grad_sync.active:
             ef = self.enc.flat
             lib.lv_txn_guard_f32(_eng.status_ptr(self.enc), _eng.status_ptr(self.dec), P(ef.grad_padded, ef.guard_index), s)
+
+    def _plain_route(self):
+        return (self.nsamples == 1 and self.objective == "elbo" and self.free_bits is None and self.enc.precision == "bf16"
+                and self.grad_sync is None and self.micro_batches == 1 and self.decoder_grads == "full")
 
     def _collective_after_bptt(self):
         return bool(self.enc.persistent and self.enc.precision == "bf16")
```

Result: no change. 12170 (median of 6 runs) (+0.9%).
